# jspenmar/slowtv_monodepth

Measured on AMD Instinct MI355X. Metric: training images/sec (640×192, 3-frame) at 1/2/4/8 MI355X; warp+SSIM HBM GB/s, higher is better.
Workload: dtype f32

## Files before the change

### include/smd_hotpath.h

```cpp
#ifndef SMD_HOTPATH_H
#define SMD_HOTPATH_H

#include <stddef.h>
#include <stdint.h>

#ifdef __cplusplus
extern "C" {
#endif

#define SMD_ABI_VERSION 8

#define SMD_OK 0
#define SMD_E_INVALID (-1)
#define SMD_E_LAUNCH (-2)
#define SMD_E_WORKSPACE (-3)
#define SMD_E_UNSUPPORTED (-4)

#define SMD_USE_MIN 0x1
#define SMD_USE_AUTOMASK 0x2
#define SMD_LOSS_L1 0x4
#define SMD_NEED_K_GRAD 0x8
#define SMD_USE_EDGES 0x10
#define SMD_LOSS_L2 0x20
#define SMD_MASK_EXPLAINABILITY 0x80
#define SMD_MASK_UNCERTAINTY 0x100
#define SMD_BWD_SKIP_DEAD_ROWS 0x400
#define SMD_BWD_NO_LIVE 0x1000
#define SMD_USE_LAPLACIAN 0x200
#define SMD_EDGES_READY 0x800
#define SMD_PACKED_READY 0x40
#define SMD_REGR_L1 0x0
#define SMD_REGR_LOG_L1 0x1
#define SMD_REGR_BERHU 0x2
#define SMD_REGR_INVERT 0x4

#define SMD_MAX_SCALES 8
#define SMD_MAX_SUPPORTS 8
#define SMD_SEL_MASKED 255

const char* smd_last_error(void);
int smd_abi_version(void);

int smd_set_knob(const char* name, int value);
void smd_reset_knobs(void);

int smd_disp_to_depth_fwd(const float* const* disp, const int* hs, const int* ws, int S, int b, int h, int w,
                          float min_depth, float max_depth, float* depth_up, float* disp_up, void* stream);
size_t smd_disp_to_depth_workspace_bytes(const int* hs, const int* ws, int S, int b, int h, int w);
int smd_disp_to_depth_bwd(const int* hs, const int* ws, int S, int b, int h, int w, float min_depth, float max_depth,
                          const float* depth_up, const float* g_depth_up, float* const* g_disp,
                          void* workspace, size_t workspace_bytes, void* stream);

size_t smd_image_recon_workspace_bytes(int b, int n, int S, int h, int w);
size_t smd_packed_supports_bytes(int b, int n, int h, int w);
int smd_image_recon_prep(const float* tgt, const float* supp, float* supp_packed, const int* hs, const int* ws, int S,
                         int b, int n, int h, int w, int flags, void* stream);
int smd_image_recon_supports_per_pass(void);
int smd_image_recon_fwd(const float* depth, const float* tgt, const float* supp, const float* T, const float* K,
                        const float* K_inv, const float* noise, uint64_t seed, float* supp_packed, float* err, uint8_t* sel, float* loss,
                        float* warp0, void* workspace, size_t workspace_bytes,
                        int b, int n, int S, int h, int w, int flags, void* stream);
int smd_image_recon_bwd(const float* depth, const float* tgt, float* supp_packed, const float* T, const float* K,
                        const float* K_inv, const uint8_t* sel, const float* g_loss,
                        float* g_depth, float* g_T, float* g_K, float* g_Kinv, void* workspace, size_t workspace_bytes,
                        int b, int n, int S, int h, int w, int flags, void* stream);

size_t smd_image_recon_disp_workspace_bytes(const int* hs, const int* ws, int S, int b, int n, int h, int w);
int smd_image_recon_disp_fwd(const float* const* disp, const int* hs, const int* ws, int S, float min_depth, float max_depth,
                             const float* tgt, const float* supp, const float* T, const float* K, const float* K_inv,
                             const float* noise, uint64_t seed, float* supp_packed, float* depth_up, float* err, uint8_t* sel, float* loss,
                             float* warp0, void* workspace, size_t workspace_bytes, int b, int n, int h, int w, int flags, void* stream);
int smd_image_recon_disp_bwd(const int* hs, const int* ws, int S, float min_depth, float max_depth, const float* depth_up,
                             float* supp_packed, const float* T, const float* K, const float* K_inv, const uint8_t* sel,
                             const float* g_loss, const float* g_depth_up_in, float* const* g_disp, float* g_T, float* g_K, float* g_Kinv,
                             void* workspace, size_t workspace_bytes, int b, int n, int h, int w, int flags, void* stream);

size_t smd_loss_path_workspace_bytes(const int* hs, const int* ws, int S, int b, int n, int h, int w);
int smd_loss_path_fwd(const float* const* disp, const int* hs, const int* ws, const int* scale_keys, int S, float min_depth, float max_depth,
                      const float* tgt, const float* supp, const float* T, const float* K, const float* K_inv, uint64_t seed,
                      float* supp_packed, float* edge_weights, float* depth_up, uint8_t* sel, float* loss3, float* stats,
                      void* workspace, size_t workspace_bytes, int b, int n, int h, int w, int flags, float w_recon, float w_smooth, void* stream);
int smd_loss_path_bwd(const float* const* disp, const int* hs, const int* ws, const int* scale_keys, int S, float min_depth, float max_depth,
                      const float* depth_up, float* supp_packed, const float* T, const float* K, const float* K_inv, const uint8_t* sel,
                      const float* stats, const float* edge_weights, const float* g_loss, float w_recon, float w_smooth,
                      const float* aa, const float* t, const uint8_t* invert, const float* fs, const float* cs,
                      float* const* g_disp, float* g_T, float* g_K, float* g_Kinv, float* g_aa, float* g_t, float* g_fs, float* g_cs,
                      void* workspace, size_t workspace_bytes, int b, int n, int h, int w, int flags, void* stream);

int smd_gaussian_blur3x3(const float* x, float* out, int planes, int h, int w, int adjoint, void* stream);
size_t smd_disp_smooth_workspace_bytes(const int* hs, const int* ws, int S, int b);
size_t smd_disp_smooth_edge_weight_bytes(const int* hs, const int* ws, int S, int b);
int smd_disp_smooth_prep(const float* img, const int* hs, const int* ws, int S, int b, int h, int w, int flags, float* edge_weights, void* stream);
int smd_disp_smooth_fwd(const float* const* disp, const int* hs, const int* ws, const int* scale_keys, int S, int b,
                        const float* img, int h, int w, int flags, float* loss, float* stats, float* disp_grad, float* image_grad,
                        float* edge_weights, void* workspace, size_t workspace_bytes, void* stream);
int smd_disp_smooth_bwd(const float* const* disp, const int* hs, const int* ws, const int* scale_keys, int S, int b,
                        const float* img, int h, int w, int flags, const float* stats, const float* edge_weights,
                        const float* g_loss, float* const* g_disp, void* stream);

size_t smd_view_synth_workspace_bytes(int B, int h, int w);
int smd_view_synth_fwd(const float* input, const float* depth, const float* T, const float* K, const float* K_inv,
                       float* warp, float* depth_warp, uint8_t* mask_valid, int B, int C, int h, int w, void* stream);
int smd_view_synth_bwd(const float* input, const float* depth, const float* T, const float* K, const float* K_inv,
                       const float* g_warp, const float* g_depth_warp,
                       float* g_input, float* g_depth, float* g_T, float* g_K, float* g_Kinv,
                       void* workspace, size_t workspace_bytes, int B, int C, int h, int w, void* stream);

size_t smd_photo_error_workspace_bytes(int N, int C, int h, int w);
int smd_photo_error_fwd(const float* pred, const float* target, float* err, int N, int C, int h, int w, int flags, float weight_ssim, void* stream);
int smd_photo_error_bwd(const float* pred, const float* target, const float* g_err, float* g_pred,
                        void* workspace, size_t workspace_bytes, int N, int C, int h, int w, int flags, float weight_ssim, void* stream);

size_t smd_regression_workspace_bytes(size_t N);
int smd_regression_fwd(const float* pred, const float* target, const uint8_t* mask, size_t N, int flags, float* loss, float* err,
                       float* stats, void* workspace, size_t workspace_bytes, void* stream);
int smd_regression_bwd(const float* pred, const float* target, const uint8_t* mask, size_t N, int flags, float* stats,
                       const float* g_loss, float* g_pred, float* g_target, void* workspace, size_t workspace_bytes, void* stream);

size_t smd_recon_reduce_workspace_bytes(int B, int h, int w);
int smd_recon_reduce_fwd(const float* err_warp, const float* err_static, const float* mask, const float* noise, uint64_t seed,
                         float* err, uint8_t* sel, float* loss, void* workspace, size_t workspace_bytes,
                         int n, int B, int h, int w, int flags, void* stream);
int smd_recon_reduce_bwd(const uint8_t* sel, const float* g_loss, float* g_err_warp, const float* err_warp, const float* err_static,
                         const float* mask, float* g_mask, int n, int B, int h, int w, int flags, void* stream);

#define SMD_GLUE_A_BF16 1
#define SMD_GLUE_SKIP_BF16 2
#define SMD_GLUE_OUT_BF16 4
size_t smd_decoder_glue_workspace_bytes(int B, int C, int h, int w);
int smd_elu_pad_fwd(const void* x, const float* bias, void* out, int B, int C, int h, int w, int apply_elu, int dtypes, void* stream);
int smd_elu_pad_bwd(const void* x, const float* bias, const void* g_out, void* g_x, float* g_bias,
                    void* workspace, size_t workspace_bytes, int B, int C, int h, int w, int apply_elu, int dtypes, void* stream);
int smd_elu_up_cat_pad_fwd(const void* a, const float* bias, const void* skip, void* out, int B, int Ca, int Cs, int h, int w, int dtypes,
                           void* stream);
int smd_elu_up_cat_pad_bwd(const void* a, const float* bias, const void* g_out, void* g_a, void* g_skip, float* g_bias,
                           void* workspace, size_t workspace_bytes, int B, int Ca, int Cs, int h, int w, int dtypes, void* stream);

#define SMD_HEAD_X_BF16 2
size_t smd_conv3x3_head_workspace_bytes(int B, int C, int h, int w);
int smd_conv3x3_head_fwd(const void* xp, const float* weight, const float* bias, float* y, int B, int C, int h, int w, int act, void* stream);
int smd_conv3x3_head_bwd(const void* xp, const float* weight, const float* y, const float* g_y, void* g_xp, float* g_weight, float* g_bias,
                         void* workspace, size_t workspace_bytes, int B, int C, int h, int w, int act, void* stream);

#define SMD_HEADN_NONE 0
#define SMD_HEADN_SIGMOID 1
#define SMD_HEADN_RELU 2
#define SMD_HEADN_X_BF16 4
size_t smd_conv3x3_headn_workspace_bytes(int B, int C, int n, int h, int w);
int smd_conv3x3_headn_fwd(const void* xp, const float* weight, const float* bias, float* y, int B, int C, int n, int h, int w, int act, void* stream);
int smd_conv3x3_headn_bwd_data(const float* weight, const float* y, const float* g_y, void* g_xp, int B, int C, int n, int h, int w, int act, void* stream);
int smd_conv3x3_headn_bwd_wgt(const void* xp, const float* y, const float* g_y, float* g_weight, float* g_bias, void* workspace, size_t workspace_bytes,
                              int B, int C, int n, int h, int w, int act, void* stream);

int smd_upsample_stack_fwd(const float* const* x, const int* hs, const int* ws, int S, int b, int n, int h, int w, float* out, void* stream);
int smd_upsample_stack_bwd(const int* hs, const int* ws, int S, int b, int n, int h, int w, const float* g_out, float* const* g_x, void* stream);

#define SMD_MEAN_BCE_ONES 0
#define SMD_MEAN_IDENTITY 1
#define SMD_MEAN_NEGATE 2
size_t smd_scale_mean_workspace_bytes(const long long* numel, int S);
int smd_scale_mean_fwd(const float* const* x, const long long* numel, int S, int mode, float* loss, void* workspace, size_t workspace_bytes, void* stream);
int smd_scale_mean_bwd(const float* const* x, const long long* numel, int S, int mode, const float* g_loss, float* const* g_x, void* stream);

size_t smd_conv3x3_thin_workspace_bytes(int B, int C, int h, int w);
int smd_conv3x3_thin_fwd(const float* xp, const float* weight, float* y, int B, int C, int h, int w, void* stream);
int smd_conv3x3_thin_bwd(const float* xp, const float* weight, const float* g_y, float* g_xp, float* g_weight, void* workspace, size_t workspace_bytes,
                         int B, int C, int h, int w, void* stream);

size_t smd_conv3x3_mfma_packed_bytes(int C, int CO, int pieces);
size_t smd_conv3x3_mfma_workspace_bytes(int B, int C, int CO, int h, int w);
int smd_conv3x3_mfma_pack(const float* weight, void* wp_fwd, void* wp_bwd, int C, int CO, int pieces, void* stream);
int smd_conv3x3_mfma_fwd(const void* xp, const void* wp_fwd, void* y, void* workspace, size_t workspace_bytes,
                         int B, int C, int CO, int h, int w, int pieces, void* stream);
int smd_conv3x3_mfma_bwd_data(const void* g_y, const void* wp_bwd, void* g_xp, void* workspace, size_t workspace_bytes,
                              int B, int C, int CO, int h, int w, int pieces, void* stream);
int smd_conv3x3_mfma_bwd_weight(const void* xp, const void* g_y, float* g_weight, void* workspace, size_t workspace_bytes,
                                int B, int C, int CO, int h, int w, int pieces, void* stream);

size_t smd_conv3x3z_mfma_workspace_bytes(int B, int C, int CO, int h, int w);
int smd_conv3x3z_mfma_fwd(const float* x, const void* wp_fwd, float* y, void* workspace, size_t workspace_bytes,
                          int B, int C, int CO, int h, int w, int pieces, void* stream);
int smd_conv3x3z_mfma_bwd_data(const float* g_y, const void* wp_bwd, float* g_x, void* workspace, size_t workspace_bytes,
                               int B, int C, int CO, int h, int w, int pieces, void* stream);
int smd_conv3x3z_mfma_bwd_weight(const float* x, const float* g_y, float* g_weight, void* workspace, size_t workspace_bytes,
                                 int B, int C, int CO, int h, int w, int pieces, void* stream);

size_t smd_conv7x7s2_packed_bytes(int C, int CO);
size_t smd_conv7x7s2_workspace_bytes(int B, int C, int CO, int H, int W);
int smd_conv7x7s2_pack(const float* weight, void* wp, int C, int CO, void* stream);
int smd_conv7x7s2_fwd(const float* x, const void* wp, float* y, int B, int C, int CO, int H, int W, void* stream);
int smd_conv7x7s2_bwd_weight(const float* x, const float* g_y, float* g_weight, void* workspace, size_t workspace_bytes,
                             int B, int C, int CO, int H, int W, void* stream);

size_t smd_bn_workspace_bytes(int N, int C, int HW);
int smd_bn_fwd(const float* x, const float* residual, const float* gamma, const float* beta, float* running_mean, float* running_var,
               float momentum, float eps, int relu, float* y, float* save_mean, float* save_invstd,
               void* workspace, size_t workspace_bytes, int N, int C, int HW, void* stream);
int smd_bn_bwd(const float* x, const float* y, const float* g_y, const float* gamma, const float* save_mean, const float* save_invstd,
               int relu, float* g_x, float* g_residual, float* g_gamma, float* g_beta,
               void* workspace, size_t workspace_bytes, int N, int C, int HW, void* stream);

int smd_maxpool3x3s2_fwd(const float* x, float* y, uint8_t* idx, int N, int C, int H, int W, void* stream);
int smd_maxpool3x3s2_bwd(const float* g_y, const uint8_t* idx, float* g_x, int N, int C, int H, int W, void* stream);

size_t smd_dwconv7x7_workspace_bytes(int C, int H, int W);
int smd_dwconv7x7_fwd(const float* x, const float* weight, const float* bias, float* y, int N, int C, int H, int W, int flip, void* stream);
int smd_dwconv7x7_wrw(const float* x, const float* g_y, float* g_weight, float* g_bias, void* workspace, size_t workspace_bytes,
                      int N, int C, int H, int W, void* stream);

size_t smd_layernorm_cf_workspace_bytes(int N, int C, int HW);
int smd_layernorm_cf_fwd(const float* x, const float* gamma, const float* beta, void* y, int y_is_bf16, float* mean, float* rstd,
                         int N, int C, int HW, float eps, void* stream);
int smd_layernorm_cf_bwd(const float* x, const void* g_y, int g_y_is_bf16, const float* gamma, const float* mean, const float* rstd,
                         float* g_x, float* g_gamma, float* g_beta, void* workspace, size_t workspace_bytes, int N, int C, int HW, void* stream);

int smd_pose_fwd(const float* aa, const float* t, const uint8_t* invert, int N, float* T, void* stream);
int smd_pose_bwd(const float* aa, const float* t, const uint8_t* invert, int N, const float* g_T, float* g_aa, float* g_t, void* stream);
int smd_intrinsics_fwd(const float* fs, const float* cs, const float* K_in, int b, int h, int w, float* K, float* K_inv, void* stream);
int smd_intrinsics_bwd(const float* fs, const float* cs, int b, int h, int w, const float* g_K, const float* g_Kinv,
                       float* g_fs, float* g_cs, void* stream);

int smd_crop_resize(const float* const* src, float* const* dst, const int* planes, int nseg, int H, int W, int crop_h, int crop_w,
                    int out_h, int out_w, const float* K_in, float* K_out, int nK, void* stream);

#define SMD_PROF_RECON_FWD 0
#define SMD_PROF_RECON_BWD 1
#define SMD_PROF_RECON_FWD_ALL 2
#define SMD_PROF_RECON_BWD_ALL 3
#define SMD_PROF_RECON_PREP 4
const char* smd_last_kernel_variant(int which);
int smd_profile_enable(int which, int capacity);
int smd_profile_collect(int which, float* ms_out, int max_out, int* n_out);

int smd_debug_stream_copy(const void* src, void* dst, size_t nbytes, int mode, void* stream);

int smd_debug_lane_shift(float* out_left, float* out_right, void* stream);

#ifdef __cplusplus
}
#endif
#endif
```

### slowtv_monodepth_amd/_lib.py

```python
from __future__ import annotations

import ctypes as C
import os
from pathlib import Path

import torch

__all__ = ['lib', 'call', 'set_knob', 'reset_knobs', 'knob_epoch', 'lib_path', 'FLAGS', 'REGR_FLAGS', 'SEL_MASKED', 'ptr_array', 'int_array', 'i64_array', 'HotpathError', 'Unsupported']

_HERE = Path(__file__).resolve().parent
lib_path = Path(os.environ.get('SMD_HOTPATH_LIB', _HERE/'libsmd_hotpath.so'))

FLAGS = {'use_min': 0x1, 'use_automask': 0x2, 'loss_l1': 0x4, 'need_k_grad': 0x8, 'use_edges': 0x10, 'loss_l2': 0x20, 'packed_ready': 0x40,
         'mask_explainability': 0x80, 'mask_uncertainty': 0x100, 'use_laplacian': 0x200, 'bwd_skip_rows': 0x400, 'edges_ready': 0x800, 'bwd_no_live': 0x1000}
REGR_FLAGS = {'l1': 0x0, 'log_l1': 0x1, 'berhu': 0x2, 'invert': 0x4}
SEL_MASKED = 255
MAX_SCALES = 8
MAX_SUPPORTS = 8

_vp, _i, _f, _sz, _u64 = C.c_void_p, C.c_int, C.c_float, C.c_size_t, C.c_uint64

PROTOTYPES = {
    'smd_last_error': (C.c_char_p, []),
    'smd_abi_version': (_i, []),
    'smd_last_kernel_variant': (C.c_char_p, [_i]),
    'smd_set_knob': (_i, [C.c_char_p, _i]),
    'smd_reset_knobs': (None, []),
    'smd_disp_to_depth_fwd': (_i, [_vp, _vp, _vp, _i, _i, _i, _i, _f, _f, _vp, _vp, _vp]),
    'smd_disp_to_depth_workspace_bytes': (_sz, [_vp, _vp, _i, _i, _i, _i]),
    'smd_disp_to_depth_bwd': (_i, [_vp, _vp, _i, _i, _i, _i, _f, _f, _vp, _vp, _vp, _vp, _sz, _vp]),
    'smd_image_recon_workspace_bytes': (_sz, [_i, _i, _i, _i, _i]),
    'smd_packed_supports_bytes': (_sz, [_i, _i, _i, _i]),
    'smd_image_recon_prep': (_i, [_vp]*5 + [_i]*6 + [_vp]),
    'smd_image_recon_supports_per_pass': (_i, []),
    'smd_image_recon_fwd': (_i, [_vp]*7 + [_u64] + [_vp]*6 + [_sz] + [_i]*6 + [_vp]),
    'smd_image_recon_bwd': (_i, [_vp]*13 + [_sz] + [_i]*6 + [_vp]),
    'smd_image_recon_disp_workspace_bytes': (_sz, [_vp, _vp, _i, _i, _i, _i, _i]),
    'smd_image_recon_disp_fwd': (_i, [_vp, _vp, _vp, _i, _f, _f] + [_vp]*6 + [_u64] + [_vp]*7 + [_sz] + [_i]*5 + [_vp]),
    'smd_image_recon_disp_bwd': (_i, [_vp, _vp, _i, _f, _f] + [_vp]*13 + [_sz] + [_i]*5 + [_vp]),
    'smd_loss_path_workspace_bytes': (_sz, [_vp, _vp, _i, _i, _i, _i, _i]),
    'smd_loss_path_fwd': (_i, [_vp]*4 + [_i, _f, _f] + [_vp]*5 + [_u64] + [_vp]*7 + [_sz] + [_i]*5 + [_f, _f, _vp]),
    'smd_loss_path_bwd': (_i, [_vp]*4 + [_i, _f, _f] + [_vp]*9 + [_f, _f] + [_vp]*14 + [_sz] + [_i]*5 + [_vp]),
    'smd_disp_smooth_workspace_bytes': (_sz, [_vp, _vp, _i, _i]),
    'smd_disp_smooth_edge_weight_bytes': (_sz, [_vp, _vp, _i, _i]),
    'smd_gaussian_blur3x3': (_i, [_vp, _vp, _i, _i, _i, _i, _vp]),
    'smd_disp_smooth_prep': (_i, [_vp, _vp, _vp, _i, _i, _i, _i, _i, _vp, _vp]),
    'smd_disp_smooth_fwd': (_i, [_vp, _vp, _vp, _vp, _i, _i, _vp, _i, _i, _i, _vp, _vp, _vp, _vp, _vp, _vp, _sz, _vp]),
    'smd_disp_smooth_bwd': (_i, [_vp, _vp, _vp, _vp, _i, _i, _vp, _i, _i, _i, _vp, _vp, _vp, _vp, _vp]),
    'smd_view_synth_workspace_bytes': (_sz, [_i, _i, _i]),
    'smd_view_synth_fwd': (_i, [_vp]*8 + [_i]*4 + [_vp]),
    'smd_view_synth_bwd': (_i, [_vp]*13 + [_sz] + [_i]*4 + [_vp]),
    'smd_photo_error_workspace_bytes': (_sz, [_i, _i, _i, _i]),
    'smd_photo_error_fwd': (_i, [_vp]*3 + [_i]*5 + [_f, _vp]),
    'smd_photo_error_bwd': (_i, [_vp]*5 + [_sz] + [_i]*5 + [_f, _vp]),
    'smd_regression_workspace_bytes': (_sz, [_sz]),
    'smd_regression_fwd': (_i, [_vp]*3 + [_sz, _i] + [_vp]*4 + [_sz, _vp]),
    'smd_regression_bwd': (_i, [_vp]*3 + [_sz, _i] + [_vp]*5 + [_sz, _vp]),
    'smd_recon_reduce_workspace_bytes': (_sz, [_i, _i, _i]),
    'smd_recon_reduce_fwd': (_i, [_vp]*4 + [_u64] + [_vp]*4 + [_sz] + [_i]*5 + [_vp]),
    'smd_recon_reduce_bwd': (_i, [_vp]*7 + [_i]*5 + [_vp]),
    'smd_decoder_glue_workspace_bytes': (_sz, [_i]*4),
    'smd_conv3x3_headn_workspace_bytes': (_sz, [_i]*5),
    'smd_conv3x3_headn_fwd': (_i, [_vp]*4 + [_i]*6 + [_vp]),
    'smd_conv3x3_headn_bwd_data': (_i, [_vp]*4 + [_i]*6 + [_vp]),
    'smd_conv3x3_headn_bwd_wgt': (_i, [_vp]*6 + [_sz] + [_i]*6 + [_vp]),
    'smd_upsample_stack_fwd': (_i, [_vp]*3 + [_i]*5 + [_vp, _vp]),
    'smd_upsample_stack_bwd': (_i, [_vp]*2 + [_i]*5 + [_vp]*3),
    'smd_scale_mean_workspace_bytes': (_sz, [_vp, _i]),
    'smd_scale_mean_fwd': (_i, [_vp]*2 + [_i]*2 + [_vp]*2 + [_sz, _vp]),
    'smd_scale_mean_bwd': (_i, [_vp]*2 + [_i]*2 + [_vp]*3),
    'smd_conv3x3_thin_workspace_bytes': (_sz, [_i]*4),
    'smd_conv3x3_thin_fwd': (_i, [_vp]*3 + [_i]*4 + [_vp]),
    'smd_conv3x3_thin_bwd': (_i, [_vp]*6 + [_sz] + [_i]*4 + [_vp]),
    'smd_conv3x3_mfma_packed_bytes': (_sz, [_i]*3),
    'smd_conv3x3_mfma_workspace_bytes': (_sz, [_i]*5),
    'smd_conv3x3_mfma_pack': (_i, [_vp]*3 + [_i]*3 + [_vp]),
    'smd_conv3x3_mfma_fwd': (_i, [_vp]*4 + [_sz] + [_i]*6 + [_vp]),
    'smd_conv3x3_mfma_bwd_data': (_i, [_vp]*4 + [_sz] + [_i]*6 + [_vp]),
    'smd_conv3x3_mfma_bwd_weight': (_i, [_vp]*4 + [_sz] + [_i]*6 + [_vp]),
    'smd_conv3x3z_mfma_workspace_bytes': (_sz, [_i]*5),
    'smd_conv3x3z_mfma_fwd': (_i, [_vp]*4 + [_sz] + [_i]*6 + [_vp]),
    'smd_conv3x3z_mfma_bwd_data': (_i, [_vp]*4 + [_sz] + [_i]*6 + [_vp]),
    'smd_conv3x3z_mfma_bwd_weight': (_i, [_vp]*4 + [_sz] + [_i]*6 + [_vp]),
    'smd_conv7x7s2_packed_bytes': (_sz, [_i]*2),
    'smd_conv7x7s2_workspace_bytes': (_sz, [_i]*5),
    'smd_conv7x7s2_pack': (_i, [_vp]*2 + [_i]*2 + [_vp]),
    'smd_conv7x7s2_fwd': (_i, [_vp]*3 + [_i]*5 + [_vp]),
    'smd_conv7x7s2_bwd_weight': (_i, [_vp]*4 + [_sz] + [_i]*5 + [_vp]),
    'smd_conv3x3_head_workspace_bytes': (_sz, [_i]*4),
    'smd_conv3x3_head_fwd': (_i, [_vp]*4 + [_i]*5 + [_vp]),
    'smd_conv3x3_head_bwd': (_i, [_vp]*8 + [_sz] + [_i]*5 + [_vp]),
    'smd_elu_pad_fwd': (_i, [_vp]*3 + [_i]*6 + [_vp]),
    'smd_elu_pad_bwd': (_i, [_vp]*6 + [_sz] + [_i]*6 + [_vp]),
    'smd_elu_up_cat_pad_fwd': (_i, [_vp]*4 + [_i]*6 + [_vp]),
    'smd_elu_up_cat_pad_bwd': (_i, [_vp]*7 + [_sz] + [_i]*6 + [_vp]),
    'smd_bn_workspace_bytes': (_sz, [_i, _i, _i]),
    'smd_bn_fwd': (_i, [_vp]*6 + [_f, _f, _i] + [_vp]*4 + [_sz] + [_i]*3 + [_vp]),
    'smd_bn_bwd': (_i, [_vp]*6 + [_i] + [_vp]*5 + [_sz] + [_i]*3 + [_vp]),
    'smd_maxpool3x3s2_fwd': (_i, [_vp]*3 + [_i]*4 + [_vp]),
    'smd_maxpool3x3s2_bwd': (_i, [_vp]*3 + [_i]*4 + [_vp]),
    'smd_dwconv7x7_workspace_bytes': (_sz, [_i]*3),
    'smd_dwconv7x7_fwd': (_i, [_vp]*4 + [_i]*5 + [_vp]),
    'smd_dwconv7x7_wrw': (_i, [_vp]*5 + [_sz] + [_i]*4 + [_vp]),
    'smd_layernorm_cf_workspace_bytes': (_sz, [_i]*3),
    'smd_layernorm_cf_fwd': (_i, [_vp]*4 + [_i] + [_vp]*2 + [_i]*3 + [_f, _vp]),
    'smd_layernorm_cf_bwd': (_i, [_vp]*2 + [_i] + [_vp]*7 + [_sz] + [_i]*3 + [_vp]),
    'smd_pose_fwd': (_i, [_vp, _vp, _vp, _i, _vp, _vp]),
    'smd_pose_bwd': (_i, [_vp, _vp, _vp, _i, _vp, _vp, _vp, _vp]),
    'smd_intrinsics_fwd': (_i, [_vp, _vp, _vp, _i, _i, _i, _vp, _vp, _vp]),
    'smd_intrinsics_bwd': (_i, [_vp, _vp, _i, _i, _i, _vp, _vp, _vp, _vp, _vp]),
    'smd_crop_resize': (_i, [_vp, _vp, _vp] + [_i]*7 + [_vp, _vp, _i, _vp]),
    'smd_profile_enable': (_i, [_i, _i]),
    'smd_profile_collect': (_i, [_i, _vp, _i, _vp]),
    'smd_debug_stream_copy': (_i, [_vp, _vp, _sz, _i, _vp]),
    'smd_debug_lane_shift': (_i, [_vp, _vp, _vp]),
}


class HotpathError(RuntimeError):
    """A call into libsmd_hotpath.so returned a negative status."""


class Unsupported(HotpathError):
    """SMD_E_UNSUPPORTED: the entry point does not serve these arguments in this build (nothing was launched); the caller takes the general operators."""


def _load() -> C.CDLL:
    if not lib_path.is_file():
        raise ImportError(
            f'{lib_path} not found: the HIP hot path is not built. Run `python -c "import __graft_entry__ as g; g.build()"` '
            f'(or `make -C slowtv_monodepth_amd/csrc`). There is no CPU/PyTorch fallback for this path.')
    handle = C.CDLL(str(lib_path))
    for name, (res, args) in PROTOTYPES.items():
        fn = getattr(handle, name)
        fn.restype, fn.argtypes = res, args
    if handle.smd_abi_version() != 8: raise ImportError(f'ABI version mismatch in {lib_path}')
    return handle


lib = _load()


def call(name: str, *args):
    rc = getattr(lib, name)(*args)
    if rc != 0:
        msg = lib.smd_last_error().decode()
        if rc == -1: raise ValueError(f'{name}: {msg}')
        if rc == -4: raise Unsupported(f'{name}: {msg}')
        raise HotpathError(f'{name} failed ({rc}): {msg}')


def set_knob(name: str, value: int) -> bool:
    global knob_epoch
    rc = lib.smd_set_knob(name.encode(), int(value))
    if rc == -1: raise ValueError(lib.smd_last_error().decode())
    knob_epoch += 1
    return rc == 0


def reset_knobs() -> None:
    global knob_epoch
    lib.smd_reset_knobs()
    knob_epoch += 1


knob_epoch = 0


def ptr_array(ptrs):
    return (C.c_void_p*len(ptrs))(*ptrs)


def int_array(vals):
    return (C.c_int*len(vals))(*[int(v) for v in vals])


def i64_array(vals):
    return (C.c_longlong*len(vals))(*[int(v) for v in vals])
```

### slowtv_monodepth_amd/conv_ops.py

```python
from __future__ import annotations

from collections import namedtuple

import torch

from . import _lib
from ._device import _check, _check_fb, _on, _ptr, _stream, _workspace, call
from .conv_routing import serve

_BF = torch.bfloat16


def _thin_bwd(xp, weight, g_y, want_x, want_w):
    if not (want_x or want_w): return None, None
    B, C, H, W = xp.shape
    g_xp = torch.empty_like(xp) if want_x else None
    g_w = torch.empty_like(weight) if want_w else None
    ws, nbytes = _workspace(xp.device, _lib.lib.smd_conv3x3_thin_workspace_bytes, B, C, H - 2, W - 2, floor=256) if want_w else (None, 0)
    call('smd_conv3x3_thin_bwd', xp.data_ptr(), weight.data_ptr(), g_y.data_ptr(), _ptr(g_xp), _ptr(g_w), _ptr(ws), nbytes, B, C, H - 2, W - 2, _stream())
    return g_xp, g_w


class _Conv3x3Thin(torch.autograd.Function):
    @staticmethod
    def forward(ctx, xp, weight):
        xp = _check('xp', xp)
        if xp.ndim != 4 or xp.shape[2] < 4 or xp.shape[3] < 4: raise ValueError(f'expected a padded (B,C,h+2,w+2) with h, w >= 2, got {tuple(xp.shape)}')
        B, C, H, W = xp.shape
        weight = _check('weight', weight, (16, C, 3, 3))
        y = torch.empty((B, 16, H - 2, W - 2), device=xp.device, dtype=torch.float32)
        call('smd_conv3x3_thin_fwd', xp.data_ptr(), weight.data_ptr(), y.data_ptr(), B, C, H - 2, W - 2, _stream())
        ctx.save_for_backward(xp, weight)
        return y

    @staticmethod
    def backward(ctx, g_y):
        xp, weight = ctx.saved_tensors
        _on(xp)
        B, C, H, W = xp.shape
        g_y = _check('grad(y)', g_y, (B, 16, H - 2, W - 2))
        return _thin_bwd(xp, weight, g_y, *ctx.needs_input_grad)


def conv3x3_thin(xp, weight):
    return _Conv3x3Thin.apply(xp, weight)


_Served = namedtuple('_Served', 'fwd data wgt thin sized')


def _served(C, CO, zpad, sized) -> _Served:
    thin = CO == 16 and C in (16, 32) and not zpad
    return _Served(fwd=(C % 16 == 0 and CO % 32 == 0) or thin,
                   data=(CO % 16 == 0 and C % 32 == 0) or (C == 16 and CO == 16 and not zpad),
                   wgt=CO % 32 == 0 or thin, thin=thin, sized=sized)


def _mfma_pack(weight, C, CO, pieces, want_fwd, want_bwd):
    nbytes = _lib.lib.smd_conv3x3_mfma_packed_bytes(C, CO, pieces)
    wf = _workspace(weight.device, nbytes, floor=256)[0] if want_fwd else None
    wb = _workspace(weight.device, nbytes, floor=256)[0] if want_bwd else None
    call('smd_conv3x3_mfma_pack', weight.data_ptr(), _ptr(wf), _ptr(wb), C, CO, pieces, _stream())
    return wf, wb


def _mfma_ws_bytes(B, C, CO, h, w, zpad):
    return (_lib.lib.smd_conv3x3z_mfma_workspace_bytes if zpad else _lib.lib.smd_conv3x3_mfma_workspace_bytes)(B, C, CO, h, w)


def _mfma_launch(entry, zpad, a, b, out, nws, dims, pieces):
    ws, nws = _workspace(out.device, nws, floor=256)
    call(('smd_conv3x3z_mfma_' if zpad else 'smd_conv3x3_mfma_') + entry, a.data_ptr(), b.data_ptr(), out.data_ptr(), ws.data_ptr(), nws, *dims, pieces, _stream())
    return out


class _Conv3x3Wide(torch.autograd.Function):
    @staticmethod
    def forward(ctx, xp, weight, pieces, force, zpad=False):
        xp = _check_fb('xp', xp)
        if zpad and xp.dtype != torch.float32: raise TypeError(f'the zero-padded convolution takes float32 tensors, got {xp.dtype}')
        if xp.ndim != 4 or (not zpad and (xp.shape[2] < 3 or xp.shape[3] < 3)):
            raise ValueError(f'expected {"(B,C,h,w)" if zpad else "a padded (B,C,h+2,w+2)"}, got {tuple(xp.shape)}')
        B, C, H, W = xp.shape
        if weight.ndim != 4 or tuple(weight.shape[1:]) != (C, 3, 3): raise ValueError(f'weight: expected (CO,{C},3,3), got {tuple(weight.shape)}')
        CO = weight.shape[0]
        weight = _check('weight', weight, (CO, C, 3, 3))
        h, w = (H, W) if zpad else (H - 2, W - 2)
        dims = (B, C, CO, h, w)
        bf = xp.dtype == _BF
        if bf: pieces = 1
        nws = _mfma_ws_bytes(*dims, zpad)
        sv = _served(C, CO, zpad, force or nws > 0)
        if force and not sv.fwd:
            raise _lib.Unsupported(f'the MFMA forward serves C % 16 == 0 with CO % 32 == 0{"" if zpad else ", or CO = 16 with C = 16 | 32"}, not C={C} CO={CO}')
        y = torch.empty((B, CO, h, w), device=xp.device, dtype=xp.dtype)
        packed = {}

        def run_mfma():
            packed['wf'], packed['wb'] = _mfma_pack(weight, C, CO, pieces, True, sv.data)
            return _mfma_launch('fwd', zpad, xp, packed['wf'], y, nws, dims, pieces)

        def run_ref():
            if zpad: return torch.conv2d(xp, weight, None, 1, 1)
            if bf: return torch.conv2d(xp, weight.to(_BF))
            if sv.thin: call('smd_conv3x3_thin_fwd', xp.data_ptr(), weight.data_ptr(), y.data_ptr(), B, C, h, w, _stream()); return y
            return torch.conv2d(xp, weight)
        op = 'fwd_z' if zpad else 'fwd_bf16' if bf else 'fwd'
        out = serve((op, *dims), run_mfma, run_ref, eligible=sv.fwd and sv.sized, force=force)
        ctx.save_for_backward(xp, weight, packed.get('wb'))
        ctx.pieces, ctx.force, ctx.zpad, ctx.served = pieces, force, zpad, sv
        return out

    @staticmethod
    def backward(ctx, g_y):
        xp, weight, wp_bwd = ctx.saved_tensors
        _on(xp)
        B, C, H, W = xp.shape
        zpad, sv = ctx.zpad, ctx.served
        CO, pieces, force = weight.shape[0], ctx.pieces, ctx.force
        h, w = (H, W) if zpad else (H - 2, W - 2)
        dims = (B, C, CO, h, w)
        need_x, need_w = ctx.needs_input_grad[0], ctx.needs_input_grad[1]
        bf = xp.dtype == _BF
        g_y = _check_fb('grad(y)', g_y.to(xp.dtype), (B, CO, h, w))
        g_xp = g_w = None
        w_ref = weight.to(_BF) if bf else weight
        pad = [1, 1] if zpad else [0, 0]
        cb = lambda mask: torch.ops.aten.convolution_backward(g_y, xp, w_ref, None, [1, 1], pad, [1, 1], False, [0, 0], 1, mask)
        thin_ref = sv.thin and not bf
        sfx = '_z' if zpad else '_bf16' if bf else ''
        nws = _mfma_ws_bytes(*dims, zpad) if sv.sized and ((need_x and sv.data) or (need_w and sv.wgt)) else 0
        if need_x:
            g_xp = torch.empty_like(xp)
            packed = {'wb': wp_bwd}

            def run_data():
                if packed['wb'] is None: packed['wb'] = _mfma_pack(weight, C, CO, pieces, False, True)[1]
                return _mfma_launch('bwd_data', zpad, g_y, packed['wb'], g_xp, nws, dims, pieces)
            ref_data = (lambda: _thin_bwd(xp, weight, g_y, True, False)[0]) if thin_ref else (lambda: cb([True, False, False])[0])
            g_xp = serve(('data' + sfx, *dims), run_data, ref_data, eligible=sv.data and sv.sized, force=force)
        if need_w:
            g_w = torch.empty_like(weight)
            run_wgt = lambda: _mfma_launch('bwd_weight', zpad, xp, g_y, g_w, nws, dims, pieces)
            ref_wgt = (lambda: _thin_bwd(xp, weight, g_y, False, True)[1]) if thin_ref else (lambda: cb([False, True, False])[1].float())
            g_w = serve(('wgt' + sfx, *dims), run_wgt, ref_wgt, eligible=sv.wgt and sv.sized, force=force)
        return g_xp, g_w, None, None, None


def conv3x3_mfma(xp, weight, pieces: int = 3):
    return _Conv3x3Wide.apply(xp, weight, int(pieces), True)


def conv3x3_wide(xp, weight):
    return _Conv3x3Wide.apply(xp, weight, 3, False)


def conv3x3_same(x, weight):
    return _Conv3x3Wide.apply(x, weight, 3, False, True)


class _Conv7x7s2Stem(torch.autograd.Function):
    @staticmethod
    def forward(ctx, x, weight):
        x = _check('x', x)
        if x.ndim != 4: raise ValueError(f'expected (B,C,H,W), got {tuple(x.shape)}')
        B, C, H, W = x.shape
        if weight.ndim != 4 or tuple(weight.shape[1:]) != (C, 7, 7): raise ValueError(f'weight: expected (CO,{C},7,7), got {tuple(weight.shape)}')
        CO = weight.shape[0]
        weight = _check('weight', weight, (CO, C, 7, 7))
        ho, wo = (H - 1)//2 + 1, (W - 1)//2 + 1
        served = _lib.lib.smd_conv7x7s2_workspace_bytes(B, C, CO, H, W) > 0
        y = torch.empty((B, CO, ho, wo), device=x.device, dtype=torch.float32)

        def run_mfma():
            wp, _ = _workspace(x.device, _lib.lib.smd_conv7x7s2_packed_bytes, C, CO)
            call('smd_conv7x7s2_pack', weight.data_ptr(), wp.data_ptr(), C, CO, _stream())
            call('smd_conv7x7s2_fwd', x.data_ptr(), wp.data_ptr(), y.data_ptr(), B, C, CO, H, W, _stream())
            return y
        y = serve(('fwd_s', B, C, CO, H, W), run_mfma, lambda: torch.conv2d(x, weight, None, 2, 3), eligible=served)
        ctx.save_for_backward(x, weight)
        ctx.served = served
        return y

    @staticmethod
    def backward(ctx, g_y):
        x, weight = ctx.saved_tensors
        dev = _on(x)
        B, C, H, W = x.shape
        CO = weight.shape[0]
        need_x, need_w = ctx.needs_input_grad
        g_y = _check('grad(y)', g_y, (B, CO, (H - 1)//2 + 1, (W - 1)//2 + 1))
        cb = lambda mask: torch.ops.aten.convolution_backward(g_y, x, weight, None, [2, 2], [3, 3], [1, 1], False, [0, 0], 1, mask)
        g_x = cb([True, False, False])[0] if need_x else None
        g_w = None
        if need_w:
            g_w = torch.empty_like(weight)

            def run_wgt():
                ws, nws = _workspace(dev, _lib.lib.smd_conv7x7s2_workspace_bytes, B, C, CO, H, W, floor=256)
                call('smd_conv7x7s2_bwd_weight', x.data_ptr(), g_y.data_ptr(), g_w.data_ptr(), ws.data_ptr(), nws, B, C, CO, H, W, _stream())
                return g_w
            g_w = serve(('wgt_s', B, C, CO, H, W), run_wgt, lambda: cb([False, True, False])[1], eligible=ctx.served)
        return g_x, g_w


def conv7x7s2_stem(x, weight):
    return _Conv7x7s2Stem.apply(x, weight)
```

### slowtv_monodepth_amd/conv_routing.py

```python
from __future__ import annotations

import torch

from ._lib import Unsupported

_MODE = 'auto'
_ROUTES: dict = {}
_AB_WARMUPS, _AB_ROUNDS, _AB_MARGIN = 2, 5, 0.97
_DECLINED = (Unsupported, ValueError)


def set_conv_route(mode: str = 'auto'):
    global _MODE
    if mode not in ('auto', 'mfma', 'miopen'): raise ValueError(mode)
    _MODE = mode
    _ROUTES.clear()


def conv_routes() -> dict:
    return dict(_ROUTES)


_COARSE_W_MAX, _COARSE_C_MIN = 80, 256
_Z_FWD_WGT = [dict(px_min=1000, ch_max=511), dict(px_min=2400)]
STATIC_RULES = {
    'padded': {'fwd': [dict(thin=True), dict(thin=False, px_min=20000, c_co_max=128*64), dict(thin=False, coarse=True, px_min=1000)],
               'data': [dict(thin=True), dict(thin=False, px_min=5000, c_max=256), dict(thin=False, coarse=True, px_min=1000)],
               'wgt': [dict(thin=False, px_min=20000, co_max=64), dict(thin=False, coarse=True, px_min=2400)]},
    'bf16': {'fwd': [dict(thin=True)], 'data': [dict(thin=True)], 'wgt': [dict(thin=True)]},
    'zpad': {'fwd': _Z_FWD_WGT, 'data': [dict(px_min=1000)], 'wgt': _Z_FWD_WGT},
    'stem': {'fwd': [dict(px_min=20000)], 'wgt': [dict(px_min=20000)]},
}
_FAMILY_OF_SUFFIX = {'': 'padded', 'bf16': 'bf16', 'z': 'zpad', 's': 'stem'}
_BOUNDS = {'px_min': lambda v, B, C, CO, h, w: B*h*w >= v,
           'c_max': lambda v, B, C, CO, h, w: C <= v,
           'co_max': lambda v, B, C, CO, h, w: CO <= v,
           'c_co_max': lambda v, B, C, CO, h, w: C*CO <= v,
           'ch_max': lambda v, B, C, CO, h, w: max(C, CO) <= v,
           'thin': lambda v, B, C, CO, h, w: (CO == 16) == v,
           'coarse': lambda v, B, C, CO, h, w: (w <= _COARSE_W_MAX and C >= _COARSE_C_MIN) == v}


def static_rule(op, B, C, CO, h, w) -> bool:
    kind, _, suffix = op.partition('_')
    clauses = STATIC_RULES[_FAMILY_OF_SUFFIX[suffix]][kind]
    return any(all(_BOUNDS[name](v, B, C, CO, h, w) for name, v in clause.items()) for clause in clauses)


_capturing = torch.cuda.is_current_stream_capturing


def _time_interleaved(run_mfma, run_ref, rounds):
    ev = [[torch.cuda.Event(enable_timing=True) for _ in range(3)] for _ in range(rounds)]
    for e in ev:
        e[0].record(); run_mfma(); e[1].record(); run_ref(); e[2].record()
    torch.cuda.synchronize()
    return [e[0].elapsed_time(e[1])*1e3 for e in ev], [e[1].elapsed_time(e[2])*1e3 for e in ev]


def _conv_route(op, B, C, CO, h, w, run_mfma, run_ref) -> bool:
    if _MODE != 'auto': return _MODE == 'mfma'
    key = (op, B, C, CO, h, w)
    r = _ROUTES.get(key)
    if r is None:
        if _capturing(): return static_rule(op, B, C, CO, h, w)
        for _ in range(_AB_WARMUPS): run_mfma(); run_ref()
        us_m, us_r = _time_interleaved(run_mfma, run_ref, _AB_ROUNDS)
        t_m, t_r = sorted(us_m)[_AB_ROUNDS//2], sorted(us_r)[_AB_ROUNDS//2]
        r = _ROUTES[key] = (t_m < _AB_MARGIN*t_r, t_m, t_r)
    return r[0]


def serve(key, run_mfma, run_ref, *, eligible, force=False):
    if not eligible: return run_ref()
    if force: return run_mfma()
    try:
        use = _conv_route(*key, run_mfma, run_ref)
    except _DECLINED:
        _ROUTES[key] = (False, float('nan'), float('nan'))
        use = False
    if use:
        try:
            return run_mfma()
        except _DECLINED:
            pass
    return run_ref()
```

### slowtv_monodepth_amd/csrc/smd_api.hip

```cpp
#include <limits.h>
#include <stdarg.h>
#include <stdio.h>
#include <stdlib.h>
#include <string.h>
#include <algorithm>

#include "smd_kernels.h"
#include "smd_smooth_dev.h"

namespace {

thread_local char g_err[512] = "";

int fail(int code, const char* fmt, ...) {
  va_list ap;
  va_start(ap, fmt);
  vsnprintf(g_err, sizeof(g_err), fmt, ap);
  va_end(ap);
  return code;
}

int check_launch(hipError_t e, const char* what) {
  if (e != hipSuccess) return fail(SMD_E_LAUNCH, "%s: %s", what, hipGetErrorString(e));
  return SMD_OK;
// ... 620 lines not shown
int smd_photo_error_bwd(const float* pred, const float* target, const float* g_err, float* g_pred, void* workspace, size_t workspace_bytes,
                        int N, int C, int h, int w, int flags, float weight_ssim, void* stream) {
  if (!pred || !target || !g_err || !g_pred || !workspace) return fail(SMD_E_INVALID, "null pointer");
  if (N < 1 || N > 65535 || C < 1 || h < 2 || w < 2) return fail(SMD_E_INVALID, "invalid sizes N=%d C=%d h=%d w=%d", N, C, h, w);
  if (workspace_bytes < smd_photo_error_workspace_bytes(N, C, h, w)) return fail(SMD_E_WORKSPACE, "workspace too small");
  if (!(weight_ssim >= 0.f && weight_ssim <= 1.f)) return fail(SMD_E_INVALID, "Invalid SSIM weight. (%g vs. [0, 1])", weight_ssim);
  return check_launch(smd::launch_photo_error_bwd(pred, target, g_err, g_pred, (float*)workspace, N, C, h, w, flags, weight_ssim, (hipStream_t)stream), "photo_error_bwd");
}

size_t smd_regression_workspace_bytes(size_t N) {
  if (N < 1) return 0;
  return align256((size_t)smd::regr_blocks(N)*3*sizeof(float));
}

int smd_regression_fwd(const float* pred, const float* target, const uint8_t* mask, size_t N, int flags, float* loss, float* err, float* stats,
                       void* workspace, size_t workspace_bytes, void* stream) {
  if (!pred || !target || !loss || !stats || !workspace) return fail(SMD_E_INVALID, "null pointer");
  if (N < 1 || N > ((size_t)1 << 40)) return fail(SMD_E_INVALID, "invalid size N=%zu", N);
  if (workspace_bytes < smd_regression_workspace_bytes(N)) return fail(SMD_E_WORKSPACE, "workspace too small");
  return check_launch(smd::launch_regression_fwd(pred, target, mask, N, flags, loss, err, stats, (float*)workspace, (hipStream_t)stream), "regression_fwd");
}

int smd_regression_bwd(const float* pred, const float* target, const uint8_t* mask, size_t N, int flags, float* stats, const float* g_loss,
                       float* g_pred, float* g_target, void* workspace, size_t workspace_bytes, void* stream) {
  if (!pred || !target || !stats || !g_loss || !workspace || (!g_pred && !g_target)) return fail(SMD_E_INVALID, "null pointer");
  if (N < 1 || N > ((size_t)1 << 40)) return fail(SMD_E_INVALID, "invalid size N=%zu", N);
  if (workspace_bytes < smd_regression_workspace_bytes(N)) return fail(SMD_E_WORKSPACE, "workspace too small");
  return check_launch(smd::launch_regression_bwd(pred, target, mask, N, flags, stats, g_loss, g_pred, g_target, (float*)workspace, (hipStream_t)stream),
                      "regression_bwd");
}

size_t smd_recon_reduce_workspace_bytes(int B, int h, int w) {
  if (B < 1 || h < 1 || w < 1) return 0;
  return align256((size_t)smd::ceil_div(B*h*w, 256)*sizeof(float));
}

int smd_recon_reduce_fwd(const float* err_warp, const float* err_static, const float* mask, const float* noise, uint64_t seed, float* err, uint8_t* sel,
                         float* loss, void* workspace, size_t workspace_bytes, int n, int B, int h, int w, int flags, void* stream) {
  if (!err_warp || !err || !sel || !loss || !workspace) return fail(SMD_E_INVALID, "null pointer");
  if ((flags & (SMD_MASK_EXPLAINABILITY | SMD_MASK_UNCERTAINTY)) && !mask) return fail(SMD_E_INVALID, "Must provide a 'mask' when masking...");
  if ((flags & SMD_USE_AUTOMASK) && !err_static) return fail(SMD_E_INVALID, "Must provide the original 'source' images when automasking...");
  if (n < 1 || n >= SMD_SEL_MASKED || B < 1 || h < 1 || w < 1) return fail(SMD_E_INVALID, "invalid sizes");
  if (workspace_bytes < smd_recon_reduce_workspace_bytes(B, h, w)) return fail(SMD_E_WORKSPACE, "workspace too small");
  return check_launch(smd::launch_recon_reduce_fwd(err_warp, err_static, mask, noise, seed, err, sel, loss, (float*)workspace, n, B, h, w, flags,
                                                   (hipStream_t)stream), "recon_reduce_fwd");
}

int smd_recon_reduce_bwd(const uint8_t* sel, const float* g_loss, float* g_err_warp, const float* err_warp, const float* err_static,
                         const float* mask, float* g_mask, int n, int B, int h, int w, int flags, void* stream) {
  if (!sel || !g_loss || !g_err_warp) return fail(SMD_E_INVALID, "null pointer");
  if (n < 1 || B < 1 || h < 1 || w < 1) return fail(SMD_E_INVALID, "invalid sizes");
  if (mask && (!g_mask || !err_warp || ((flags & SMD_USE_AUTOMASK) && !err_static))) return fail(SMD_E_INVALID, "a masked reduction needs err_warp, err_static (with automask) and g_mask");
  return check_launch(smd::launch_recon_reduce_bwd(sel, g_loss, g_err_warp, err_warp, err_static, mask, g_mask, n, B, h, w, flags, (hipStream_t)stream), "recon_reduce_bwd");
}

static bool dec_sizes_ok(long long planes, int h, int w) {
  return planes >= 1 && h >= 2 && w >= 2 && (long long)(h + 2)*(w + 2) < (1ll << 30) && planes*(((long long)(h + 2)*(w + 2) + 255)/256) < (1ll << 31);
}
size_t smd_decoder_glue_workspace_bytes(int B, int C, int h, int w) {
  if (B < 1 || C < 1 || h < 1 || w < 1) return 0;
  return align256(smd::decoder_bias_partials(B, C, h, w)*sizeof(float));
}
int smd_elu_pad_fwd(const void* x, const float* bias, void* out, int B, int C, int h, int w, int apply_elu, int dtypes, void* stream) {
  if (!x || !out) return fail(SMD_E_INVALID, "null pointer");
  if (B < 1 || C < 1 || !dec_sizes_ok((long long)B*C, h, w)) return fail(SMD_E_INVALID, "invalid sizes B=%d C=%d h=%d w=%d", B, C, h, w);
  return check_launch(smd::launch_elu_pad_fwd(x, bias, out, B, C, h, w, apply_elu, dtypes, (hipStream_t)stream), "elu_pad_fwd");
}
int smd_elu_pad_bwd(const void* x, const float* bias, const void* g_out, void* g_x, float* g_bias, void* workspace, size_t workspace_bytes,
                    int B, int C, int h, int w, int apply_elu, int dtypes, void* stream) {
  if (!x || !g_out || !g_x || (g_bias && !workspace)) return fail(SMD_E_INVALID, "null pointer");
  if (B < 1 || C < 1 || !dec_sizes_ok((long long)B*C, h, w)) return fail(SMD_E_INVALID, "invalid sizes B=%d C=%d h=%d w=%d", B, C, h, w);
  if (g_bias && workspace_bytes < smd_decoder_glue_workspace_bytes(B, C, h, w)) return fail(SMD_E_WORKSPACE, "workspace too small");
  return check_launch(smd::launch_elu_pad_bwd(x, bias, g_out, g_x, g_bias, (float*)workspace, B, C, h, w, apply_elu, dtypes, (hipStream_t)stream), "elu_pad_bwd");
}
static bool head_sizes_ok(int B, int C, int h, int w) {
  return B >= 1 && C >= 1 && C < 65535 && dec_sizes_ok((long long)B*C, h, w) && (long long)B*((h + 47)/48) < 65536 && h < 65536 && (long long)B*C*(h + 2)*(w + 2) < (1ll << 40);
}
size_t smd_conv3x3_head_workspace_bytes(int B, int C, int h, int w) {
  if (!head_sizes_ok(B, C, h, w)) return 0;
  return align256(smd::conv_head_partials(B, C, h, w)*sizeof(float));
}
int smd_conv3x3_head_fwd(const void* xp, const float* weight, const float* bias, float* y, int B, int C, int h, int w, int act, void* stream) {
  if (!xp || !weight || !y) return fail(SMD_E_INVALID, "null pointer");
  if (!head_sizes_ok(B, C, h, w) || (act & ~(1 | SMD_HEAD_X_BF16))) return fail(SMD_E_INVALID, "invalid sizes B=%d C=%d h=%d w=%d act=%d", B, C, h, w, act);
  return check_launch(smd::launch_conv_head_fwd(xp, (act & SMD_HEAD_X_BF16) != 0, weight, bias, y, B, C, h, w, act & 1, (hipStream_t)stream), "conv3x3_head_fwd");
}
int smd_conv3x3_head_bwd(const void* xp, const float* weight, const float* y, const float* g_y, void* g_xp, float* g_weight, float* g_bias,
                         void* workspace, size_t workspace_bytes, int B, int C, int h, int w, int act, void* stream) {
  if (!weight || !y || !g_y || (!g_xp && !g_weight) || (g_weight && (!xp || !workspace)) || (g_bias && !g_weight)) return fail(SMD_E_INVALID, "null pointer");
  if (!head_sizes_ok(B, C, h, w) || (act & ~(1 | SMD_HEAD_X_BF16))) return fail(SMD_E_INVALID, "invalid sizes B=%d C=%d h=%d w=%d act=%d", B, C, h, w, act);
  if (g_weight && workspace_bytes < smd_conv3x3_head_workspace_bytes(B, C, h, w)) return fail(SMD_E_WORKSPACE, "workspace too small");
  return check_launch(smd::launch_conv_head_bwd(xp, (act & SMD_HEAD_X_BF16) != 0, weight, y, g_y, g_xp, g_weight, g_bias, (float*)workspace, B, C, h, w, act & 1, (hipStream_t)stream), "conv3x3_head_bwd");
}
static bool headn_args_ok(int B, int C, int n, int h, int w, int act) {
  const int a = act & 3;
  return n >= 1 && n <= 4 && head_sizes_ok(B, C, h, w) && (act & ~(3 | SMD_HEADN_X_BF16)) == 0 && a != 3 && dec_sizes_ok((long long)B*n, h, w);
}
size_t smd_conv3x3_headn_workspace_bytes(int B, int C, int n, int h, int w) {
  if (!headn_args_ok(B, C, n, h, w, 0)) return 0;
  return align256(smd::conv_headn_partials(B, C, n, h, w)*sizeof(float));
}
int smd_conv3x3_headn_fwd(const void* xp, const float* weight, const float* bias, float* y, int B, int C, int n, int h, int w, int act, void* stream) {
  if (!xp || !weight || !y) return fail(SMD_E_INVALID, "null pointer");
  if (!headn_args_ok(B, C, n, h, w, act)) return fail(SMD_E_INVALID, "invalid sizes B=%d C=%d n=%d h=%d w=%d act=%d (1 <= n <= 4)", B, C, n, h, w, act);
  return check_launch(smd::launch_conv_headn_fwd(xp, (act & SMD_HEADN_X_BF16) != 0, weight, bias, y, B, C, n, h, w, act & 3, (hipStream_t)stream), "conv3x3_headn_fwd");
}
int smd_conv3x3_headn_bwd_data(const float* weight, const float* y, const float* g_y, void* g_xp, int B, int C, int n, int h, int w, int act, void* stream) {
  if (!weight || !y || !g_y || !g_xp) return fail(SMD_E_INVALID, "null pointer");
  if (!headn_args_ok(B, C, n, h, w, act)) return fail(SMD_E_INVALID, "invalid sizes B=%d C=%d n=%d h=%d w=%d act=%d (1 <= n <= 4)", B, C, n, h, w, act);
  return check_launch(smd::launch_conv_headn_bwd(nullptr, (act & SMD_HEADN_X_BF16) != 0, weight, y, g_y, g_xp, nullptr, nullptr, nullptr, B, C, n, h, w, act & 3,
                                                 (hipStream_t)stream), "conv3x3_headn_bwd_data");
}
int smd_conv3x3_headn_bwd_wgt(const void* xp, const float* y, const float* g_y, float* g_weight, float* g_bias, void* workspace, size_t workspace_bytes,
                              int B, int C, int n, int h, int w, int act, void* stream) {
  if (!xp || !y || !g_y || !g_weight || !workspace) return fail(SMD_E_INVALID, "null pointer");
  if (!headn_args_ok(B, C, n, h, w, act)) return fail(SMD_E_INVALID, "invalid sizes B=%d C=%d n=%d h=%d w=%d act=%d (1 <= n <= 4)", B, C, n, h, w, act);
  if (workspace_bytes < smd_conv3x3_headn_workspace_bytes(B, C, n, h, w)) return fail(SMD_E_WORKSPACE, "workspace too small");
  return check_launch(smd::launch_conv_headn_bwd(xp, (act & SMD_HEADN_X_BF16) != 0, nullptr, y, g_y, nullptr, g_weight, g_bias, (float*)workspace, B, C, n, h, w, act & 3,
                                                 (hipStream_t)stream), "conv3x3_headn_bwd_wgt");
}

static int up_stack_check(int S, int b, int n, int h, int w) {
  if (b < 1 || n < 1 || h < 1 || w < 1 || (long long)b*n > 65535 || (long long)h*w >= (1ll << 30)) return fail(SMD_E_INVALID, "invalid sizes b=%d n=%d h=%d w=%d (b*n <= 65535)", b, n, h, w);
  if ((long long)S*b*n*h*w >= (1ll << 40)) return fail(SMD_E_INVALID, "output too large");
  return SMD_OK;
}
int smd_upsample_stack_fwd(const float* const* x, const int* hs, const int* ws, int S, int b, int n, int h, int w, float* out, void* stream) {
  if (!x || !out) return fail(SMD_E_INVALID, "null pointer");
  if (int rc = up_stack_check(S, b, n, h, w)) return rc;
  smd::ScaleSet sc;
  if (int rc = fill_scales(sc, x, nullptr, hs, ws, nullptr, S)) return rc;
  for (int s = 0; s < S; ++s) {
    if (!x[s]) return fail(SMD_E_INVALID, "null input pointer for scale %d", s);
    if ((long long)hs[s]*ws[s] >= (1ll << 30)) return fail(SMD_E_INVALID, "scale %d too large", s);
  }
  return check_launch(smd::launch_upsample_stack_fwd(sc, b*n, h, w, out, (hipStream_t)stream), "upsample_stack_fwd");
}
int smd_upsample_stack_bwd(const int* hs, const int* ws, int S, int b, int n, int h, int w, const float* g_out, float* const* g_x, void* stream) {
  if (!g_out || !g_x) return fail(SMD_E_INVALID, "null pointer");
  if (int rc = up_stack_check(S, b, n, h, w)) return rc;
  smd::ScaleSet sc;
  if (int rc = fill_scales(sc, nullptr, g_x, hs, ws, nullptr, S)) return rc;
  long long blocks = 0;
  for (int s = 0; s < S; ++s) {
    if (!g_x[s]) return fail(SMD_E_INVALID, "null gradient pointer for scale %d", s);
    if ((long long)hs[s]*ws[s] >= (1ll << 30)) return fail(SMD_E_INVALID, "scale %d too large", s);
    blocks += ((long long)hs[s]*ws[s] + 255)/256;
  }
  if (blocks >= (1ll << 31)) return fail(SMD_E_INVALID, "too many source pixels");
  return check_launch(smd::launch_upsample_stack_bwd(sc, b*n, h, w, g_out, (hipStream_t)stream), "upsample_stack_bwd");
}
static int fill_means(smd::MeanSet& ms, const float* const* x, float* const* g, const long long* numel, int S, int mode) {
  if (S < 1 || S > SMD_MAX_SCALES) return fail(SMD_E_INVALID, "S=%d outside [1, %d]", S, SMD_MAX_SCALES);
  if (!numel) return fail(SMD_E_INVALID, "null size array");
  if (mode < SMD_MEAN_BCE_ONES || mode > SMD_MEAN_NEGATE) return fail(SMD_E_INVALID, "invalid mode %d", mode);
  memset(&ms, 0, sizeof(ms));
  ms.S = S;
  for (int s = 0; s < S; ++s) {
    if (numel[s] < 1) return fail(SMD_E_INVALID, "scale %d is empty", s);
    ms.p[s] = x ? x[s] : nullptr; ms.g[s] = g ? g[s] : nullptr; ms.n[s] = numel[s];
  }
  if (smd::scale_mean_blocks(ms) < 1) return fail(SMD_E_INVALID, "too many elements");
  return SMD_OK;
}
size_t smd_scale_mean_workspace_bytes(const long long* numel, int S) {
  smd::MeanSet ms;
  if (fill_means(ms, nullptr, nullptr, numel, S, 0)) return 0;
  return 256 + align256((size_t)ms.first_block[SMD_MAX_SCALES]*sizeof(float));
}
int smd_scale_mean_fwd(const float* const* x, const long long* numel, int S, int mode, float* loss, void* workspace, size_t workspace_bytes, void* stream) {
  if (!x || !loss || !workspace) return fail(SMD_E_INVALID, "null pointer");
  smd::MeanSet ms;
  if (int rc = fill_means(ms, x, nullptr, numel, S, mode)) return rc;
  for (int s = 0; s < S; ++s) if (!x[s]) return fail(SMD_E_INVALID, "null input pointer for scale %d", s);
  if (workspace_bytes < smd_scale_mean_workspace_bytes(numel, S)) return fail(SMD_E_WORKSPACE, "workspace too small");
  return check_launch(smd::launch_scale_mean_fwd(ms, mode, (float*)((char*)workspace + 256), (unsigned*)workspace, loss, (hipStream_t)stream), "scale_mean_fwd");
}
int smd_scale_mean_bwd(const float* const* x, const long long* numel, int S, int mode, const float* g_loss, float* const* g_x, void* stream) {
  if (!g_loss || !g_x || (mode == SMD_MEAN_BCE_ONES && !x)) return fail(SMD_E_INVALID, "null pointer");
  smd::MeanSet ms;
  if (int rc = fill_means(ms, x, g_x, numel, S, mode)) return rc;
  for (int s = 0; s < S; ++s) if (!g_x[s] || (mode == SMD_MEAN_BCE_ONES && !x[s])) return fail(SMD_E_INVALID, "null pointer for scale %d", s);
  return check_launch(smd::launch_scale_mean_bwd(ms, mode, g_loss, (hipStream_t)stream), "scale_mean_bwd");
}
static bool thin_sizes_ok(int B, int C, int h, int w) { return (C == 16 || C == 32) && head_sizes_ok(B, C, h, w) && dec_sizes_ok((long long)B*16, h, w) && B < 65536 && h + 2 < 4*65536; }
size_t smd_conv3x3_thin_workspace_bytes(int B, int C, int h, int w) {
  if (!thin_sizes_ok(B, C, h, w)) return 0;
  return align256(smd::conv_thin_partials(B, C, h, w)*sizeof(float));
}
int smd_conv3x3_thin_bwd(const float* xp, const float* weight, const float* g_y, float* g_xp, float* g_weight, void* workspace, size_t workspace_bytes,
                         int B, int C, int h, int w, void* stream) {
  if (!g_y || (!g_xp && !g_weight) || (g_xp && !weight) || (g_weight && (!xp || !workspace))) return fail(SMD_E_INVALID, "null pointer");
  if (C != 16 && C != 32 && C >= 1) return fail(SMD_E_UNSUPPORTED, "the thin convolution serves 16 or 32 input channels, not %d", C);
  if (!thin_sizes_ok(B, C, h, w)) return fail(SMD_E_INVALID, "invalid sizes B=%d C=%d h=%d w=%d", B, C, h, w);
  if (g_weight && workspace_bytes < smd_conv3x3_thin_workspace_bytes(B, C, h, w)) return fail(SMD_E_WORKSPACE, "workspace too small");
  hipStream_t st = (hipStream_t)stream;
  if (g_xp) { if (int rc = check_launch(smd::launch_conv_thin_bwd_data(g_y, weight, g_xp, B, C, h, w, st), "conv3x3_thin_bwd (data)")) return rc; }
  if (g_weight) { if (int rc = check_launch(smd::launch_conv_thin_bwd_wgt(xp, g_y, g_weight, (float*)workspace, B, C, h, w, st), "conv3x3_thin_bwd (weights)")) return rc; }
  return SMD_OK;
}
int smd_conv3x3_thin_fwd(const float* xp, const float* weight, float* y, int B, int C, int h, int w, void* stream) {
  if (!xp || !weight || !y) return fail(SMD_E_INVALID, "null pointer");
  if (C != 16 && C != 32 && C >= 1) return fail(SMD_E_UNSUPPORTED, "the thin convolution serves 16 or 32 input channels, not %d", C);
  if (!thin_sizes_ok(B, C, h, w)) return fail(SMD_E_INVALID, "invalid sizes B=%d C=%d h=%d w=%d", B, C, h, w);
  return check_launch(smd::launch_conv_thin_fwd(xp, weight, y, B, C, h, w, (hipStream_t)stream), "conv3x3_thin_fwd");
}
static bool mfma_sizes_ok(int B, int C, int CO, int h, int w) {
  return B >= 1 && C >= 1 && CO >= 1 && C <= 4096 && CO <= 4096 && h >= 1 && w >= 1 && h < 32768 && w < 32768 && (long long)(h + 2)*(w + 2) < (1ll << 30) &&
         (long long)B*((C + 31)/32)*((CO + 31)/32) < 65536 && (long long)C*(h + 2)*(w + 2) < (1ll << 29) && (long long)CO*h*w < (1ll << 29);
}
using smd::ConvOp;
static bool conv_two_tiles() { return knob("conv_two_tiles", 0) != 0; }
size_t smd_conv3x3_mfma_packed_bytes(int C, int CO, int pieces) {
  if (C < 1 || CO < 1 || pieces < 1 || pieces > 3) return 0;
  return align256(smd::conv_mfma_packed_elems(C, CO, pieces)*2);
}
static size_t mfma_workspace_bytes(bool zpad, int B, int C, int CO, int h, int w, bool two_tiles) {
  if (!mfma_sizes_ok(B, C, CO, h, w)) return 0;
  size_t n = std::max({(size_t)64, smd::conv_mfma_split_elems(ConvOp::Fwd, zpad, B, C, CO, h, w, two_tiles), smd::conv_mfma_split_elems(ConvOp::Data, zpad, B, C, CO, h, w, two_tiles)});
  if (smd::conv_mfma_served(ConvOp::Wgt, zpad, C, CO)) n = std::max(n, smd::conv_mfma_wgrad_partials(zpad, B, C, CO, h, w));
  return align256(n*sizeof(float));
}
size_t smd_conv3x3_mfma_workspace_bytes(int B, int C, int CO, int h, int w) { return mfma_workspace_bytes(false, B, C, CO, h, w, conv_two_tiles()); }
size_t smd_conv3x3z_mfma_workspace_bytes(int B, int C, int CO, int h, int w) { return mfma_workspace_bytes(true, B, C, CO, h, w, conv_two_tiles()); }
static int mfma_unserved(ConvOp op, bool zpad, int C, int CO) {
  const char* name[] = {"forward", "data gradient", "weight gradient"};
  return fail(SMD_E_UNSUPPORTED, "the %s%s does not serve C=%d CO=%d", zpad ? "zero-padded " : "", name[(int)op], C, CO);
}
static int mfma_check(ConvOp op, bool zpad, size_t workspace_bytes, int B, int C, int CO, int h, int w, int pieces, bool two_tiles) {
  if (zpad && pieces != 2 && pieces != 3) return fail(SMD_E_UNSUPPORTED, "the zero-padded forms take float tensors: pieces 2 or 3, not %d", pieces);
  if (pieces < 1 || pieces > 3) return fail(SMD_E_UNSUPPORTED, "pieces must be 1 (bfloat16 tensors), 2 or 3 (float tensors), not %d", pieces);
  if (!mfma_sizes_ok(B, C, CO, h, w)) return fail(SMD_E_INVALID, "invalid sizes B=%d C=%d CO=%d h=%d w=%d", B, C, CO, h, w);
  if (!smd::conv_mfma_served(op, zpad, C, CO)) return mfma_unserved(op, zpad, C, CO);
  if (workspace_bytes < mfma_workspace_bytes(zpad, B, C, CO, h, w, two_tiles)) return fail(SMD_E_WORKSPACE, "workspace too small");
  return SMD_OK;
}
int smd_conv3x3_mfma_pack(const float* weight, void* wp_fwd, void* wp_bwd, int C, int CO, int pieces, void* stream) {
  if (!weight || (!wp_fwd && !wp_bwd)) return fail(SMD_E_INVALID, "null pointer");
  if (pieces < 1 || pieces > 3) return fail(SMD_E_UNSUPPORTED, "pieces must be 1 (bfloat16 tensors), 2 or 3 (float tensors), not %d", pieces);
  if (C < 1 || CO < 1 || C > 4096 || CO > 4096) return fail(SMD_E_INVALID, "invalid sizes C=%d CO=%d", C, CO);
  if (wp_fwd && !smd::conv_mfma_served(ConvOp::Fwd, false, C, CO)) return mfma_unserved(ConvOp::Fwd, false, C, CO);
  if (wp_bwd && !smd::conv_mfma_served(ConvOp::Data, false, C, CO)) return mfma_unserved(ConvOp::Data, false, C, CO);
  return check_launch(smd::launch_conv_mfma_pack(weight, wp_fwd, wp_bwd, C, CO, pieces, (hipStream_t)stream), "conv3x3_mfma_pack");
}
static int mfma_form(ConvOp op, bool zpad, const void* in, const void* wp, void* out, void* workspace, size_t workspace_bytes, int B, int C, int CO, int h, int w, int pieces, void* stream, const char* what) {
  if (!in || !wp || !out || !workspace) return fail(SMD_E_INVALID, "null pointer");
  const bool two_tiles = conv_two_tiles();
  if (int rc = mfma_check(op, zpad, workspace_bytes, B, C, CO, h, w, pieces, two_tiles)) return rc;
  const auto launch = op == ConvOp::Fwd ? smd::launch_conv_mfma_fwd : smd::launch_conv_mfma_bwd_data;
  return check_launch(launch(in, wp, out, (float*)workspace, zpad, B, C, CO, h, w, pieces, two_tiles, (hipStream_t)stream), what);
}
static int mfma_bwd_weight(bool zpad, const void* x, const void* g_y, float* g_weight, void* workspace, size_t workspace_bytes, int B, int C, int CO, int h, int w, int pieces, void* stream) {
  if (!x || !g_y || !g_weight || !workspace) return fail(SMD_E_INVALID, "null pointer");
  if (int rc = mfma_check(ConvOp::Wgt, zpad, workspace_bytes, B, C, CO, h, w, pieces, conv_two_tiles())) return rc;
  return check_launch(smd::launch_conv_mfma_bwd_wgt(x, g_y, g_weight, (float*)workspace, zpad, B, C, CO, h, w, pieces, (hipStream_t)stream), zpad ? "conv3x3z_mfma_bwd_weight" : "conv3x3_mfma_bwd_weight");
}
int smd_conv3x3_mfma_fwd(const void* xp, const void* wp_fwd, void* y, void* workspace, size_t workspace_bytes, int B, int C, int CO, int h, int w, int pieces, void* stream) {
  return mfma_form(ConvOp::Fwd, false, xp, wp_fwd, y, workspace, workspace_bytes, B, C, CO, h, w, pieces, stream, "conv3x3_mfma_fwd");
}
int smd_conv3x3_mfma_bwd_data(const void* g_y, const void* wp_bwd, void* g_xp, void* workspace, size_t workspace_bytes, int B, int C, int CO, int h, int w, int pieces, void* stream) {
  return mfma_form(ConvOp::Data, false, g_y, wp_bwd, g_xp, workspace, workspace_bytes, B, C, CO, h, w, pieces, stream, "conv3x3_mfma_bwd_data");
}
int smd_conv3x3_mfma_bwd_weight(const void* xp, const void* g_y, float* g_weight, void* workspace, size_t workspace_bytes, int B, int C, int CO, int h, int w, int pieces, void* stream) {
  return mfma_bwd_weight(false, xp, g_y, g_weight, workspace, workspace_bytes, B, C, CO, h, w, pieces, stream);
}
int smd_conv3x3z_mfma_fwd(const float* x, const void* wp_fwd, float* y, void* workspace, size_t workspace_bytes, int B, int C, int CO, int h, int w, int pieces, void* stream) {
  return mfma_form(ConvOp::Fwd, true, x, wp_fwd, y, workspace, workspace_bytes, B, C, CO, h, w, pieces, stream, "conv3x3z_mfma_fwd");
}
int smd_conv3x3z_mfma_bwd_data(const float* g_y, const void* wp_bwd, float* g_x, void* workspace, size_t workspace_bytes, int B, int C, int CO, int h, int w, int pieces, void* stream) {
  return mfma_form(ConvOp::Data, true, g_y, wp_bwd, g_x, workspace, workspace_bytes, B, C, CO, h, w, pieces, stream, "conv3x3z_mfma_bwd_data");
}
int smd_conv3x3z_mfma_bwd_weight(const float* x, const float* g_y, float* g_weight, void* workspace, size_t workspace_bytes, int B, int C, int CO, int h, int w, int pieces, void* stream) {
  return mfma_bwd_weight(true, x, g_y, g_weight, workspace, workspace_bytes, B, C, CO, h, w, pieces, stream);
}
static bool stem_sizes_ok(int B, int C, int H, int W) {
  if (B < 1 || B > 65535 || C < 1 || H < 1 || W < 1) return false;
  const long long ho = (H - 1)/2 + 1, wo = (W - 1)/2 + 1;
  return (long long)C*H*W < (1ll << 31) && 64*ho*wo < (1ll << 31) && (ho + 3)/4 <= 65535;
}
size_t smd_conv7x7s2_packed_bytes(int C, int CO) { return smd::conv_stem_served(C, CO) ? smd::conv_stem_packed_bytes(C) : 0; }
size_t smd_conv7x7s2_workspace_bytes(int B, int C, int CO, int H, int W) {
  if (!smd::conv_stem_served(C, CO) || !stem_sizes_ok(B, C, H, W)) return 0;
  return align256(smd::conv_stem_wgrad_floats(B, C, H, W)*sizeof(float));
}
int smd_conv7x7s2_pack(const float* weight, void* wp, int C, int CO, void* stream) {
  if (!weight || !wp) return fail(SMD_E_INVALID, "null pointer");
  if (!smd::conv_stem_served(C, CO)) return fail(SMD_E_UNSUPPORTED, "the stem kernels serve CO == 64 with C == 3 | 6, not C=%d CO=%d", C, CO);
  return check_launch(smd::launch_conv_stem_pack(weight, wp, C, (hipStream_t)stream), "conv7x7s2_pack");
}
int smd_conv7x7s2_fwd(const float* x, const void* wp, float* y, int B, int C, int CO, int H, int W, void* stream) {
  if (!x || !wp || !y) return fail(SMD_E_INVALID, "null pointer");
  if (!smd::conv_stem_served(C, CO)) return fail(SMD_E_UNSUPPORTED, "the stem kernels serve CO == 64 with C == 3 | 6, not C=%d CO=%d", C, CO);
  if (!stem_sizes_ok(B, C, H, W)) return fail(SMD_E_INVALID, "invalid sizes B=%d C=%d H=%d W=%d", B, C, H, W);
  return check_launch(smd::launch_conv_stem_fwd(x, wp, y, B, C, H, W, (hipStream_t)stream), "conv7x7s2_fwd");
}
int smd_conv7x7s2_bwd_weight(const float* x, const float* g_y, float* g_weight, void* workspace, size_t workspace_bytes,
                             int B, int C, int CO, int H, int W, void* stream) {
  if (!x || !g_y || !g_weight || !workspace) return fail(SMD_E_INVALID, "null pointer");
  if (!smd::conv_stem_served(C, CO)) return fail(SMD_E_UNSUPPORTED, "the stem kernels serve CO == 64 with C == 3 | 6, not C=%d CO=%d", C, CO);
  if (!stem_sizes_ok(B, C, H, W)) return fail(SMD_E_INVALID, "invalid sizes B=%d C=%d H=%d W=%d", B, C, H, W);
  if (workspace_bytes < smd_conv7x7s2_workspace_bytes(B, C, CO, H, W)) return fail(SMD_E_WORKSPACE, "workspace too small");
  return check_launch(smd::launch_conv_stem_bwd_wgt(x, g_y, g_weight, (float*)workspace, B, C, H, W, (hipStream_t)stream), "conv7x7s2_bwd_weight");
}
int smd_elu_up_cat_pad_fwd(const void* a, const float* bias, const void* skip, void* out, int B, int Ca, int Cs, int h, int w, int dtypes, void* stream) {
  if (!a || !out || (Cs > 0 && !skip)) return fail(SMD_E_INVALID, "null pointer");
  if (B < 1 || Ca < 1 || Cs < 0 || h < 1 || w < 1 || !dec_sizes_ok((long long)B*(Ca + Cs), 2*h, 2*w))
    return fail(SMD_E_INVALID, "invalid sizes B=%d Ca=%d Cs=%d h=%d w=%d", B, Ca, Cs, h, w);
  return check_launch(smd::launch_elu_up_cat_pad_fwd(a, bias, skip, out, B, Ca, Cs, h, w, dtypes, (hipStream_t)stream), "elu_up_cat_pad_fwd");
}
int smd_elu_up_cat_pad_bwd(const void* a, const float* bias, const void* g_out, void* g_a, void* g_skip, float* g_bias,
                           void* workspace, size_t workspace_bytes, int B, int Ca, int Cs, int h, int w, int dtypes, void* stream) {
  if (!a || !g_out || (!g_a && !g_skip) || (g_bias && (!workspace || !g_a))) return fail(SMD_E_INVALID, "null pointer");
  if (B < 1 || Ca < 1 || Cs < 0 || h < 1 || w < 1 || !dec_sizes_ok((long long)B*(Ca + Cs), 2*h, 2*w))
    return fail(SMD_E_INVALID, "invalid sizes B=%d Ca=%d Cs=%d h=%d w=%d", B, Ca, Cs, h, w);
  if (g_bias && workspace_bytes < smd_decoder_glue_workspace_bytes(B, Ca, h, w)) return fail(SMD_E_WORKSPACE, "workspace too small");
  return check_launch(smd::launch_elu_up_cat_pad_bwd(a, bias, g_out, g_a, g_skip, g_bias, (float*)workspace, B, Ca, Cs, h, w, dtypes, (hipStream_t)stream),
                      "elu_up_cat_pad_bwd");
}

size_t smd_bn_workspace_bytes(int N, int C, int HW) {
  if (N < 1 || C < 1 || HW < 1) return 0;
  return align256(((size_t)C*smd::bn_chunks(N, HW)*2 + (size_t)C*3)*sizeof(float));
}
int smd_bn_fwd(const float* x, const float* residual, const float* gamma, const float* beta, float* running_mean, float* running_var,
               float momentum, float eps, int relu, float* y, float* save_mean, float* save_invstd, void* workspace, size_t workspace_bytes,
               int N, int C, int HW, void* stream) {
  if (!x || !gamma || !beta || !y || !save_mean || !save_invstd || !workspace) return fail(SMD_E_INVALID, "null pointer");
  if (N < 1 || C < 1 || C > 65535 || HW < 1 || (long long)N*HW < 2) return fail(SMD_E_INVALID, "invalid sizes N=%d C=%d HW=%d", N, C, HW);
  if (workspace_bytes < smd_bn_workspace_bytes(N, C, HW)) return fail(SMD_E_WORKSPACE, "workspace too small");
  return check_launch(smd::launch_bn_fwd(x, residual, gamma, beta, running_mean, running_var, momentum, eps, relu, y, save_mean, save_invstd,
                                         (float*)workspace, N, C, HW, (hipStream_t)stream), "bn_fwd");
}
int smd_bn_bwd(const float* x, const float* y, const float* g_y, const float* gamma, const float* save_mean, const float* save_invstd, int relu,
               float* g_x, float* g_residual, float* g_gamma, float* g_beta, void* workspace, size_t workspace_bytes, int N, int C, int HW,
               void* stream) {
  if (!x || !g_y || !gamma || !save_mean || !save_invstd || !g_x || !g_gamma || !g_beta || !workspace || (relu && !y))
    return fail(SMD_E_INVALID, "null pointer");
  if (N < 1 || C < 1 || C > 65535 || HW < 1) return fail(SMD_E_INVALID, "invalid sizes N=%d C=%d HW=%d", N, C, HW);
  if (workspace_bytes < smd_bn_workspace_bytes(N, C, HW)) return fail(SMD_E_WORKSPACE, "workspace too small");
  return check_launch(smd::launch_bn_bwd(x, y, g_y, gamma, save_mean, save_invstd, relu, g_x, g_residual, g_gamma, g_beta, (float*)workspace,
                                         N, C, HW, (hipStream_t)stream), "bn_bwd");
}

int smd_maxpool3x3s2_fwd(const float* x, float* y, uint8_t* idx, int N, int C, int H, int W, void* stream) {
  if (!x || !y || !idx) return fail(SMD_E_INVALID, "null pointer");
  if (N < 1 || C < 1 || H < 1 || W < 1 || (long long)N*C*(((long long)H*W + 1023)/1024) >= (1ll << 31)) return fail(SMD_E_INVALID, "invalid sizes");
  return check_launch(smd::launch_maxpool_fwd(x, y, idx, (size_t)N*C, H, W, (hipStream_t)stream), "maxpool_fwd");
}
int smd_maxpool3x3s2_bwd(const float* g_y, const uint8_t* idx, float* g_x, int N, int C, int H, int W, void* stream) {
  if (!g_y || !idx || !g_x) return fail(SMD_E_INVALID, "null pointer");
  if (N < 1 || C < 1 || H < 1 || W < 1 || (long long)N*C*(((long long)H*W + 1023)/1024) >= (1ll << 31)) return fail(SMD_E_INVALID, "invalid sizes");
  return check_launch(smd::launch_maxpool_bwd(g_y, idx, g_x, (size_t)N*C, H, W, (hipStream_t)stream), "maxpool_bwd");
}

static bool dw_sizes_ok(int N, int C, int H, int W) {
  return N >= 1 && C >= 1 && H >= 1 && W >= 1 && (long long)N*C*smd::dwconv_tiles(H, W) < (1ll << 31) && (long long)H*W < (1ll << 30);
}
size_t smd_dwconv7x7_workspace_bytes(int C, int H, int W) {
  if (C < 1 || H < 1 || W < 1) return 0;
  return align256((size_t)C*smd::dwconv_tiles(H, W)*50*sizeof(float));
}
int smd_dwconv7x7_fwd(const float* x, const float* weight, const float* bias, float* y, int N, int C, int H, int W, int flip, void* stream) {
  if (!x || !weight || !y) return fail(SMD_E_INVALID, "null pointer");
  if (!dw_sizes_ok(N, C, H, W)) return fail(SMD_E_INVALID, "invalid sizes N=%d C=%d H=%d W=%d", N, C, H, W);
  return check_launch(smd::launch_dwconv7(x, weight, bias, y, N, C, H, W, flip, (hipStream_t)stream), "dwconv7x7_fwd");
}
int smd_dwconv7x7_wrw(const float* x, const float* g_y, float* g_weight, float* g_bias, void* workspace, size_t workspace_bytes,
                      int N, int C, int H, int W, void* stream) {
  if (!x || !g_y || !g_weight || !workspace) return fail(SMD_E_INVALID, "null pointer");
  if (!dw_sizes_ok(N, C, H, W)) return fail(SMD_E_INVALID, "invalid sizes N=%d C=%d H=%d W=%d", N, C, H, W);
  if (workspace_bytes < smd_dwconv7x7_workspace_bytes(C, H, W)) return fail(SMD_E_WORKSPACE, "workspace too small");
  return check_launch(smd::launch_dwconv7_wrw(x, g_y, g_weight, g_bias, (float*)workspace, N, C, H, W, (hipStream_t)stream), "dwconv7x7_wrw");
}

size_t smd_layernorm_cf_workspace_bytes(int N, int C, int HW) {
  if (N < 1 || C < 1 || HW < 1) return 0;
  return align256((size_t)smd::ln_cf_chunks((size_t)N*HW)*C*2*sizeof(float));
}
int smd_layernorm_cf_fwd(const float* x, const float* gamma, const float* beta, void* y, int y_is_bf16, float* mean, float* rstd, int N, int C, int HW,
                         float eps, void* stream) {
  if (!x || !gamma || !beta || !y || !mean || !rstd) return fail(SMD_E_INVALID, "null pointer");
  if (N < 1 || C < 1 || HW < 1 || (long long)N*HW >= (1ll << 38)) return fail(SMD_E_INVALID, "invalid sizes N=%d C=%d HW=%d", N, C, HW);
  return check_launch(smd::launch_ln_cf_fwd(x, gamma, beta, y, y_is_bf16, mean, rstd, N, C, HW, eps, (hipStream_t)stream), "layernorm_cf_fwd");
}
int smd_layernorm_cf_bwd(const float* x, const void* g_y, int g_y_is_bf16, const float* gamma, const float* mean, const float* rstd, float* g_x, float* g_gamma,
                         float* g_beta, void* workspace, size_t workspace_bytes, int N, int C, int HW, void* stream) {
  if (!x || !g_y || !gamma || !mean || !rstd || !g_x || !g_gamma || !g_beta || !workspace) return fail(SMD_E_INVALID, "null pointer");
  if (N < 1 || C < 1 || C > 32767 || HW < 1) return fail(SMD_E_INVALID, "invalid sizes N=%d C=%d HW=%d", N, C, HW);
  if (workspace_bytes < smd_layernorm_cf_workspace_bytes(N, C, HW)) return fail(SMD_E_WORKSPACE, "workspace too small");
  return check_launch(smd::launch_ln_cf_bwd(x, g_y, g_y_is_bf16, gamma, mean, rstd, g_x, g_gamma, g_beta, (float*)workspace, N, C, HW, (hipStream_t)stream),
                      "layernorm_cf_bwd");
}

int smd_pose_fwd(const float* aa, const float* t, const uint8_t* invert, int N, float* T, void* stream) {
  if (!aa || !t || !T) return fail(SMD_E_INVALID, "null pointer");
  if (N < 1) return fail(SMD_E_INVALID, "invalid size N=%d", N);
  return check_launch(smd::launch_pose_fwd(aa, t, invert, N, T, (hipStream_t)stream), "pose_fwd");
}
int smd_pose_bwd(const float* aa, const float* t, const uint8_t* invert, int N, const float* g_T, float* g_aa, float* g_t, void* stream) {
  if (!aa || !t || !g_T || !g_aa || !g_t) return fail(SMD_E_INVALID, "null pointer");
  if (N < 1) return fail(SMD_E_INVALID, "invalid size N=%d", N);
  return check_launch(smd::launch_pose_bwd(aa, t, invert, N, g_T, g_aa, g_t, (hipStream_t)stream), "pose_bwd");
}
int smd_intrinsics_fwd(const float* fs, const float* cs, const float* K_in, int b, int h, int w, float* K, float* K_inv, void* stream) {
  if (!K_inv || (fs && (!cs || !K)) || (!fs && !K_in)) return fail(SMD_E_INVALID, "null pointer");
  if (b < 1 || h < 1 || w < 1) return fail(SMD_E_INVALID, "invalid sizes");
  return check_launch(smd::launch_intrinsics_fwd(fs, cs, K_in, b, h, w, K, K_inv, (hipStream_t)stream), "intrinsics_fwd");
}
int smd_intrinsics_bwd(const float* fs, const float* cs, int b, int h, int w, const float* g_K, const float* g_Kinv,
                       float* g_fs, float* g_cs, void* stream) {
  if (!fs || !cs || !g_K || !g_Kinv || !g_fs || !g_cs) return fail(SMD_E_INVALID, "null pointer");
  if (b < 1 || h < 1 || w < 1) return fail(SMD_E_INVALID, "invalid sizes");
  return check_launch(smd::launch_intrinsics_bwd(fs, cs, b, h, w, g_K, g_Kinv, g_fs, g_cs, (hipStream_t)stream), "intrinsics_bwd");
}

int smd_crop_resize(const float* const* src, float* const* dst, const int* planes, int nseg, int H, int W, int crop_h, int crop_w,
                    int out_h, int out_w, const float* K_in, float* K_out, int nK, void* stream) {
  if (!src || !dst || !planes) return fail(SMD_E_INVALID, "null pointer");
  if (nseg < 1 || nseg > smd::SMD_MAX_AR_SEGMENTS) return fail(SMD_E_INVALID, "nseg=%d outside [1, %d]", nseg, smd::SMD_MAX_AR_SEGMENTS);
  if (H < 2 || W < 2 || crop_h < 1 || crop_w < 1 || crop_h > H || crop_w > W || out_h < 1 || out_w < 1)
    return fail(SMD_E_INVALID, "invalid sizes: input %dx%d, crop %dx%d, output %dx%d", H, W, crop_h, crop_w, out_h, out_w);
  if ((K_in != nullptr) != (K_out != nullptr) || (K_in && nK < 1)) return fail(SMD_E_INVALID, "K_in / K_out / nK must be given together");
  smd::CropResizeArgs a;
  memset(&a, 0, sizeof(a));
  long long total = 0;
  for (int k = 0; k < nseg; ++k) {
    if (!src[k] || !dst[k] || planes[k] < 1) return fail(SMD_E_INVALID, "segment %d: null pointer or no planes", k);
    a.src[k] = src[k]; a.dst[k] = dst[k]; a.planes[k] = planes[k]; a.first_plane[k] = (int)total;
    total += planes[k];
  }
  if (total + 1 > 65535) return fail(SMD_E_INVALID, "too many image planes for one launch (%lld)", total);
  a.nseg = nseg; a.H = H; a.W = W; a.ch = crop_h; a.cw = crop_w; a.oh = out_h; a.ow = out_w;
  a.y0 = (int)((double)H/2.0 - (double)crop_h/2.0); a.x0 = (int)((double)W/2.0 - (double)crop_w/2.0);
  a.resample = (crop_h != H || crop_w != W) ? 1 : 0;
  a.K_in = K_in; a.K_out = K_out; a.nK = nK;
  return check_launch(smd::launch_crop_resize(a, (hipStream_t)stream), "crop_resize");
}

int smd_profile_enable(int which, int capacity) {
  if (which < 0 || which > 4 || capacity < 0) return fail(SMD_E_INVALID, "bad profile slot");
  ProfSlot& p = g_prof[which];
  for (int i = 0; i < 2*p.cap; ++i) (void)hipEventDestroy(p.ev[i]);
  delete[] p.ev;
  p = ProfSlot();
  if (capacity == 0) return SMD_OK;
  p.ev = new hipEvent_t[2*capacity];
  for (int i = 0; i < 2*capacity; ++i)
    if (hipEventCreate(&p.ev[i]) != hipSuccess) return fail(SMD_E_LAUNCH, "hipEventCreate failed");
  p.cap = capacity;
  return SMD_OK;
}

int smd_profile_collect(int which, float* ms_out, int max_out, int* n_out) {
  if (which < 0 || which > 4 || !ms_out || !n_out) return fail(SMD_E_INVALID, "bad profile arguments");
  ProfSlot& p = g_prof[which];
  int n = 0;
  for (int i = 0; i < p.used && n < max_out; ++i) {
    if (hipEventSynchronize(p.ev[2*i + 1]) != hipSuccess) return fail(SMD_E_LAUNCH, "hipEventSynchronize failed");
    float ms = 0.f;
    if (hipEventElapsedTime(&ms, p.ev[2*i], p.ev[2*i + 1]) != hipSuccess) return fail(SMD_E_LAUNCH, "hipEventElapsedTime failed");
    ms_out[n++] = ms;
  }
  p.used = 0;
  *n_out = n;
  return SMD_OK;
}

int smd_debug_stream_copy(const void* src, void* dst, size_t nbytes, int mode, void* stream) {
  if (!src || !dst) return fail(SMD_E_INVALID, "null pointer");
  if (nbytes < 16 || (nbytes & 15) || ((uintptr_t)src & 15) || ((uintptr_t)dst & 15)) return fail(SMD_E_INVALID, "size and pointers must be multiples of 16");
  return check_launch(smd::launch_stream_copy(src, dst, nbytes, mode, (hipStream_t)stream), "stream_copy");
}

int smd_debug_lane_shift(float* out_left, float* out_right, void* stream) {
  if (!out_left || !out_right) return fail(SMD_E_INVALID, "null pointer");
  return check_launch(smd::launch_debug_lane_shift(out_left, out_right, (hipStream_t)stream), "debug_lane_shift");
}

}
```

### slowtv_monodepth_amd/csrc/smd_conv_mfma.hip

```cpp
#include "smd_common.h"
#include "smd_kernels.h"
#include "smd_split_dev.h"
#include <algorithm>
#include <type_traits>

namespace smd {

template <int P> __device__ __forceinline__ void split_pair(unsigned short a, unsigned short b, unsigned (&p)[P]) {
  static_assert(P == 1, "bfloat16 operands have one piece");
  p[0] = (unsigned)a | ((unsigned)b << 16);
}
template <typename T> struct RawOf { typedef float type; };
template <> struct RawOf<bf16> { typedef unsigned short type; };
template <typename T> __device__ __forceinline__ void store_out(T* p, size_t i, float v);
template <> __device__ __forceinline__ void store_out<float>(float* p, size_t i, float v) { p[i] = v; }
template <> __device__ __forceinline__ void store_out<bf16>(bf16* p, size_t i, float v) { p[i] = __float2bfloat16(v); }

template <int P>
__global__ __launch_bounds__(256) void k_conv_pack_w(const float* __restrict__ w, unsigned short* __restrict__ wp_fwd, unsigned short* __restrict__ wp_bwd, int CO, int C) {
  const int idx = blockIdx.x*256 + threadIdx.x;
  if (idx >= CO*C*9) return;
  const int tap = idx % 9, c = (idx/9) % C, co = idx/(9*C);
  unsigned pk[P];
  split_pair<P>(w[idx], 0.f, pk);
// ... 812 lines not shown
  bf16x8 A[3][P];
#pragma unroll
  for (int r = 0; r < 3; ++r)
#pragma unroll
    for (int p = 0; p < P; ++p) A[r][p] = as_frag(uint4{0u, 0u, 0u, 0u});

  auto step = [&](int i, bf16x8 (&a0)[P], const bf16x8 (&a1)[P], const bf16x8 (&a2)[P]) {
    const int after = min(D - 2, nsteps - 1 - i);
    if (after >= 2) asm volatile("s_waitcnt vmcnt(%0)" :: "n"(2*NDMA) : "memory");
    else if (after == 1) asm volatile("s_waitcnt vmcnt(%0)" :: "n"(NDMA) : "memory");
    else asm volatile("s_waitcnt vmcnt(0)" ::: "memory");
    __builtin_amdgcn_s_barrier();
    asm volatile("" ::: "memory");
    if (i + D - 1 < nsteps) issue(i + D - 1);
    const float* slot = reinterpret_cast<const float*>(lds) + (i % D)*SLOT;
    const float* xr = slot + (nc*16 + j)*CS + ks*32 + q*8;
    const float* gr = slot + XDW + j*CS + ks*32 + q*8;
    const float4 x0v = *reinterpret_cast<const float4*>(xr), x1v = *reinterpret_cast<const float4*>(xr + 4);
    const float2 x2v = *reinterpret_cast<const float2*>(xr + 8);
    const float4 g0v = *reinterpret_cast<const float4*>(gr), g1v = *reinterpret_cast<const float4*>(gr + 4);
    unsigned px[5][P], pg[4][P];
    split_pair<P>(x0v.x, x0v.y, px[0]); split_pair<P>(x0v.z, x0v.w, px[1]); split_pair<P>(x1v.x, x1v.y, px[2]); split_pair<P>(x1v.z, x1v.w, px[3]); split_pair<P>(x2v.x, x2v.y, px[4]);
    split_pair<P>(g0v.x, g0v.y, pg[0]); split_pair<P>(g0v.z, g0v.w, pg[1]); split_pair<P>(g1v.x, g1v.y, pg[2]); split_pair<P>(g1v.z, g1v.w, pg[3]);
    bf16x8 Bx[3][P];
#pragma unroll
    for (int p = 0; p < P; ++p) {
      Bx[0][p] = as_frag(uint4{px[0][p], px[1][p], px[2][p], px[3][p]});
      Bx[1][p] = as_frag(uint4{__builtin_amdgcn_alignbit(px[1][p], px[0][p], 16), __builtin_amdgcn_alignbit(px[2][p], px[1][p], 16),
                               __builtin_amdgcn_alignbit(px[3][p], px[2][p], 16), __builtin_amdgcn_alignbit(px[4][p], px[3][p], 16)});
      Bx[2][p] = as_frag(uint4{px[1][p], px[2][p], px[3][p], px[4][p]});
      a0[p] = as_frag(i < nrows ? uint4{pg[0][p], pg[1][p], pg[2][p], pg[3][p]} : uint4{0u, 0u, 0u, 0u});
    }
#pragma unroll
    for (int ky = 0; ky < 3; ++ky) {
      const bf16x8 (&a)[P] = ky == 0 ? a0 : ky == 1 ? a1 : a2;
#pragma unroll
      for (int t = 0; t < NPROD; ++t)
#pragma unroll
        for (int kx = 0; kx < 3; ++kx) acc[ky*3 + kx] = __builtin_amdgcn_mfma_f32_16x16x32_bf16(a[prod_a(P, t)], Bx[kx][prod_b(P, t)], acc[ky*3 + kx], 0, 0, 0);
    }
  };

  static_assert(D == 4, "the waits above");
#pragma unroll
  for (int r = 0; r < D - 1; ++r) issue(r);
  for (int i = 0; i < nsteps; i += 3) {
    step(i, A[0], A[2], A[1]);
    if (i + 1 < nsteps) step(i + 1, A[1], A[0], A[2]);
    if (i + 2 < nsteps) step(i + 2, A[2], A[1], A[0]);
  }
  __syncthreads();
  float* red = reinterpret_cast<float*>(lds);
  if (ks == 1) {
#pragma unroll
    for (int t = 0; t < 9; ++t)
#pragma unroll
      for (int v = 0; v < 4; ++v) red[(nc*36 + t*4 + v)*64 + lane] = acc[t][v];
  }
  __syncthreads();
  if (ks == 0) {
    const size_t blk = ((size_t)b*gridDim.y + blockIdx.y)*gridDim.x + blockIdx.x;
#pragma unroll
    for (int t = 0; t < 9; ++t)
#pragma unroll
      for (int v = 0; v < 4; ++v) {
        const int co = 4*q + v, c = nc*16 + j;
        partial[((blk*9 + t)*16 + co)*C + c] = acc[t][v] + red[(nc*36 + t*4 + v)*64 + lane];
      }
  }
}

template <bool DIRECT>
__global__ __launch_bounds__(256) void k_conv_wgrad_finalize(const float* __restrict__ partial, unsigned T, unsigned G, int CO, int C, double* __restrict__ slice, float* __restrict__ g_w) {
  __shared__ double part[4][64];
  const int lane = threadIdx.x & 63, wv = threadIdx.x >> 6;
  const int n = CO*C*9, i = blockIdx.x*64 + lane;
  const unsigned g = blockIdx.y, t0 = (unsigned)(((unsigned long long)T*g)/G), t1 = (unsigned)(((unsigned long long)T*(g + 1))/G);
  double s = 0.0;
  if (i < n) for (unsigned t = t0 + wv; t < t1; t += 4) s += (double)partial[(size_t)t*n + i];
  part[wv][lane] = s;
  __syncthreads();
  if (wv == 0 && i < n) {
    const double tot = (part[0][lane] + part[1][lane]) + (part[2][lane] + part[3][lane]);
    if (DIRECT) { const int c = i % C, co = (i/C) % CO, tap = i/(C*CO); g_w[((size_t)co*C + c)*9 + tap] = (float)tot; }
    else slice[(size_t)g*n + i] = tot;
  }
}
__global__ __launch_bounds__(256) void k_conv_wgrad_finalize2(const double* __restrict__ slice, unsigned G, int CO, int C, float* __restrict__ g_w) {
  const int n = CO*C*9, i = blockIdx.x*256 + threadIdx.x;
  if (i >= n) return;
  double tot = 0.0;
  unsigned g = 0;
  for (; g + 8 <= G; g += 8) {
    double v[8];
#pragma unroll
    for (int k = 0; k < 8; ++k) v[k] = slice[(size_t)(g + k)*n + i];
#pragma unroll
    for (int k = 0; k < 8; ++k) tot += v[k];
  }
  for (; g < G; ++g) tot += slice[(size_t)g*n + i];
  const int c = i % C, co = (i/C) % CO, tap = i/(C*CO);
  g_w[((size_t)co*C + c)*9 + tap] = (float)tot;
}
static unsigned wgrad_slices(unsigned T) { return T < 64 ? 1u : std::min(32u, T/16); }

static void wgrad_shape(int B, int C, int CO, int h, int w, dim3& grid, int& rows, int& spb, bool multi) {
  const int cgs = ceil_div(C, 64)*(CO/32), strips = ceil_div(w, 32), base = strips*B*cgs;
  const int groups = std::max(1, std::min(512/std::max(base, 1), ceil_div(h, 12)));
  rows = ceil_div(h, groups);
  spb = 1;
  if (multi && rows == h && base > 512) {
    const long long per = (long long)strips*cgs;
    long long best = -1;
    for (int s = 1; s <= B; ++s) {
      const long long nsg = ceil_div(B, s), cost = ceil_div(nsg*per, 256ll)*(s*(h + 2) + 4);
      if (s > 1 && nsg*per < 512) break;
      if (best < 0 || cost < best) { best = cost; spb = s; }
    }
  }
  grid = dim3(strips, ceil_div(h, rows), ceil_div(B, spb)*cgs);
}
static void wgrad_shape(int B, int C, int CO, int h, int w, dim3& grid, int& rows) { int spb; wgrad_shape(B, C, CO, h, w, grid, rows, spb, false); }
static void wgrad16_shape(int B, int C, int h, int w, dim3& grid, int& rows) {
  const int strips = ceil_div(w, 64);
  const long long units = (long long)strips*B, slots = C == 16 ? 1024 : 768;
  const int groups = (int)std::max(1ll, std::min<long long>(ceil_div(h, 12), slots/units));
  rows = ceil_div(h, groups);
  grid = dim3(strips, ceil_div(h, rows), B);
}
static unsigned wgrad_sets(int B, int C, int CO, int h, int w, bool multi) {
  dim3 grid; int rows, spb = 1;
  if (CO == 16) wgrad16_shape(B, C, h, w, grid, rows); else wgrad_shape(B, C, CO, h, w, grid, rows, spb, multi);
  return grid.x*grid.y*(unsigned)ceil_div(B, spb);
}
static size_t wgrad_floats(unsigned T, int C, int CO) {
  const size_t n = (size_t)9*CO*C;
  const unsigned G = wgrad_slices(T);
  return (size_t)T*n + (G > 1 ? 2*(size_t)G*n : 0);
}
size_t conv_mfma_wgrad_partials(bool zpad, int B, int C, int CO, int h, int w) { return wgrad_floats(wgrad_sets(B, C, CO, h, w, zpad), C, CO); }
static size_t thin_packed_elems(int C, int pieces) { return (size_t)(C >> 4)*5*pieces*512; }
size_t conv_mfma_packed_elems(int C, int CO, int pieces) { return std::max((size_t)CO*C*9*pieces, CO == 16 ? thin_packed_elems(C, pieces) : (size_t)0); }

#define SMD_BY_PIECES(pieces, CALL) do { if ((pieces) == 3) { CALL(3, float); } else if ((pieces) == 2) { CALL(2, float); } else { CALL(1, bf16); } } while (0)

template <int P, typename T>
static void launch_conv16(const void* in, const void* wp, void* out, int B, int CK, bool bwd, int hi, int wi, int ho, int wo, hipStream_t st) {
  const unsigned gx = ceil_div(wo, 64), gy = ceil_div(ho, 4), gz = B;
  const dim3 grid(8*(unsigned)ceil_div((long long)gx*gy*gz, 8ll));
  const uint4* wq = (const uint4*)wp;
  const T* i_ = (const T*)in; T* o_ = (T*)out;
  if (bwd) hipLaunchKernelGGL((k_conv16_mfma<1, P, true, T, T>), grid, dim3(256), 0, st, i_, wq, o_, hi, wi, ho, wo, gx, gy, gz);
  else if (CK == 16) hipLaunchKernelGGL((k_conv16_mfma<1, P, false, T, T>), grid, dim3(256), 0, st, i_, wq, o_, hi, wi, ho, wo, gx, gy, gz);
  else hipLaunchKernelGGL((k_conv16_mfma<2, P, false, T, T>), grid, dim3(256), 0, st, i_, wq, o_, hi, wi, ho, wo, gx, gy, gz);
}

hipError_t launch_conv_mfma_pack(const float* w, void* wp_fwd, void* wp_bwd, int C, int CO, int pieces, hipStream_t st) {
  if (CO == 16) {
    void* thin_bwd = (C == 16) ? wp_bwd : nullptr;
    if (wp_fwd || thin_bwd) {
      const dim3 g16(ceil_div((C >> 4)*5*512, 256));
#define SMD_CALL(P, T) hipLaunchKernelGGL((k_conv_pack_w16<P>), g16, dim3(256), 0, st, w, (unsigned short*)wp_fwd, (unsigned short*)thin_bwd, C)
      SMD_BY_PIECES(pieces, SMD_CALL);
#undef SMD_CALL
    }
    if (C == 16 || !wp_bwd) return hipGetLastError();
    wp_fwd = nullptr;
  }
  const dim3 grid(ceil_div(CO*C*9, 256));
#define SMD_CALL(P, T) hipLaunchKernelGGL((k_conv_pack_w<P>), grid, dim3(256), 0, st, w, (unsigned short*)wp_fwd, (unsigned short*)wp_bwd, CO, C)
  SMD_BY_PIECES(pieces, SMD_CALL);
#undef SMD_CALL
  return hipGetLastError();
}

struct ConvShape { int TC, TRB, NM, KS, kcs, S; unsigned gx, gy, gz; dim3 grid; size_t out_elems; };
static double band_shape(int B, int CK, int ho, int wo, int& BR, int& S) {
  constexpr int NP = ConvTile<0>::NPIX;
  const int PW = wo + 2;
  if (3*PW > NP || (long long)B*CK*(ho + 2)*PW >= (1ll << 31)) return 0.0;
  if (ho*wo <= 128) {
    BR = ho; S = std::min(256/(ho*wo), B);
    while (S > 1 && S*(ho + 2)*PW > NP) --S;
  } else {
    S = 1; BR = std::min(ho, 256/wo);
    while (BR > 0 && (BR + 2)*PW > NP) --BR;
    if (BR == 0) return 0.0;
  }
  return (double)B*ho*wo/((double)ceil_div(ho, BR)*ceil_div(B, S)*256.0);
}
static ConvShape conv_shape(int B, int CK, int M, int ho, int wo, bool two_tiles) {
  ConvShape s;
  s.TC = wo >= 48 ? 64 : 32; s.TRB = wo >= 48 ? 4 : 8; s.S = 1;
  const int KC = CK >> 4;
  {
    const double rect = (double)B*ho*wo/((double)ceil_div(wo, s.TC)*s.TC*ceil_div(ho, s.TRB)*s.TRB*B);
    int BR = 0, S = 1;
    const double band = rect < 0.9 ? band_shape(B, CK, ho, wo, BR, S) : 0.0;
    if (band > rect + 0.05) {
      s.TC = 0; s.TRB = BR; s.S = S; s.NM = 1;
      s.gx = BR; s.gy = ceil_div(ho, BR); s.gz = ceil_div(B, S);
      s.out_elems = (size_t)B*M*ho*wo;
      const long long base = (long long)s.gy*s.gz*(M/32);
      double best = -1.0;
      for (int kcs = std::min(2, KC); kcs <= KC; ++kcs) {
        const int KS = ceil_div(KC, kcs);
        if (ceil_div(KC, KS) != kcs) continue;
        const double cost = (double)ceil_div(base*KS, 512ll)*(kcs + 1) + (KS > 1 ? (2.0*KS + 1.0)*s.out_elems*4.0/25e6 : 0.0);
        if (best < 0.0 || cost < best - 1e-9) { best = cost; s.kcs = kcs; s.KS = KS; }
      }
      s.grid = dim3(8*(unsigned)ceil_div(base*s.KS, 8ll));
      return s;
    }
  }
  const long long tiles = (long long)ceil_div(wo, s.TC)*ceil_div(ho, s.TRB)*B;
  s.NM = (M % 64 == 0 && tiles*(M/64) >= 256 && two_tiles) ? 2 : 1;
  const long long base = tiles*(M/(32*s.NM));
  int ks = 1;
  if (base < 384) ks = (int)std::min<long long>(std::max(KC/2, 1), (512 + base - 1)/base);
  s.kcs = ceil_div(KC, ks); s.KS = ceil_div(KC, s.kcs);
  s.gx = ceil_div(wo, s.TC); s.gy = ceil_div(ho, s.TRB); s.gz = B;
  s.grid = dim3(8*(unsigned)ceil_div((long long)s.gx*s.gy*s.gz*(M/(32*s.NM))*s.KS, 8ll));
  s.out_elems = (size_t)B*M*ho*wo;
  return s;
}
size_t conv_mfma_split_elems(ConvOp op, bool zpad, int B, int C, int CO, int h, int w, bool two_tiles) {
  if (op == ConvOp::Wgt || !conv_mfma_served(op, zpad, C, CO) || (CO == 16 && (op == ConvOp::Fwd || C == 16))) return 0;
  const int e = zpad ? 0 : 2;
  const ConvShape s = op == ConvOp::Fwd ? conv_shape(B, C, CO, h, w, two_tiles) : conv_shape(B, CO, C, h + e, w + e, two_tiles);
  return s.KS > 1 ? (size_t)s.KS*s.out_elems : 0;
}

template <int P, int OFF, typename T>
static void launch_conv_form(const void* in, const void* wp, void* out, float* split_ws, int B, int CK, int M, int hi, int wi, int ho, int wo, bool two_tiles, hipStream_t st) {
  const ConvShape s = conv_shape(B, CK, M, ho, wo, two_tiles);
  const uint4* wq = (const uint4*)wp;
  const T* i_ = (const T*)in;
  T* dst = s.KS > 1 ? reinterpret_cast<T*>(split_ws) : (T*)out;
  if (s.TC == 0) hipLaunchKernelGGL((k_conv_mfma<0, P, OFF, T, T, 1>), s.grid, dim3(256), 0, st, i_, wq, dst, CK, M, hi, wi, ho, wo, s.KS, s.kcs, s.out_elems, s.gx, s.gy, s.gz, s.S, B);
  else if (s.NM == 2) {
    if (s.TC == 64) hipLaunchKernelGGL((k_conv_mfma<64, P, OFF, T, T, 2>), s.grid, dim3(512), 0, st, i_, wq, dst, CK, M, hi, wi, ho, wo, s.KS, s.kcs, s.out_elems, s.gx, s.gy, s.gz, 1, B);
    else hipLaunchKernelGGL((k_conv_mfma<32, P, OFF, T, T, 2>), s.grid, dim3(512), 0, st, i_, wq, dst, CK, M, hi, wi, ho, wo, s.KS, s.kcs, s.out_elems, s.gx, s.gy, s.gz, 1, B);
  } else if (s.TC == 64) hipLaunchKernelGGL((k_conv_mfma<64, P, OFF, T, T, 1>), s.grid, dim3(256), 0, st, i_, wq, dst, CK, M, hi, wi, ho, wo, s.KS, s.kcs, s.out_elems, s.gx, s.gy, s.gz, 1, B);
  else hipLaunchKernelGGL((k_conv_mfma<32, P, OFF, T, T, 1>), s.grid, dim3(256), 0, st, i_, wq, dst, CK, M, hi, wi, ho, wo, s.KS, s.kcs, s.out_elems, s.gx, s.gy, s.gz, 1, B);
  if (s.KS > 1) {
    const size_t n4 = s.out_elems/4;
    hipLaunchKernelGGL((k_conv_split_sum<T>), dim3((unsigned)((n4 + 255)/256)), dim3(256), 0, st, split_ws, (T*)out, n4, s.KS);
  }
}

#define SMD_BY_PIECES_F32(pieces, CALL) do { if ((pieces) == 3) { CALL(3); } else { CALL(2); } } while (0)
hipError_t launch_conv_mfma_fwd(const void* x, const void* wp_fwd, void* y, float* split_ws, bool zpad, int B, int C, int CO, int h, int w, int pieces, bool two_tiles, hipStream_t st) {
  if (zpad) {
#define SMD_CALL(P) launch_conv_form<P, 1, float>(x, wp_fwd, y, split_ws, B, C, CO, h, w, h, w, two_tiles, st)
    SMD_BY_PIECES_F32(pieces, SMD_CALL);
#undef SMD_CALL
  } else if (CO == 16) {
#define SMD_CALL(P, T) launch_conv16<P, T>(x, wp_fwd, y, B, C, false, h + 2, w + 2, h, w, st)
    SMD_BY_PIECES(pieces, SMD_CALL);
#undef SMD_CALL
  } else {
#define SMD_CALL(P, T) launch_conv_form<P, 0, T>(x, wp_fwd, y, split_ws, B, C, CO, h + 2, w + 2, h, w, two_tiles, st)
    SMD_BY_PIECES(pieces, SMD_CALL);
#undef SMD_CALL
  }
  return hipGetLastError();
}
hipError_t launch_conv_mfma_bwd_data(const void* gy, const void* wp_bwd, void* g_x, float* split_ws, bool zpad, int B, int C, int CO, int h, int w, int pieces, bool two_tiles, hipStream_t st) {
  if (zpad) {
#define SMD_CALL(P) launch_conv_form<P, 1, float>(gy, wp_bwd, g_x, split_ws, B, CO, C, h, w, h, w, two_tiles, st)
    SMD_BY_PIECES_F32(pieces, SMD_CALL);
#undef SMD_CALL
  } else if (CO == 16 && C == 16) {
#define SMD_CALL(P, T) launch_conv16<P, T>(gy, wp_bwd, g_x, B, 16, true, h, w, h + 2, w + 2, st)
    SMD_BY_PIECES(pieces, SMD_CALL);
#undef SMD_CALL
  } else {
#define SMD_CALL(P, T) launch_conv_form<P, 2, T>(gy, wp_bwd, g_x, split_ws, B, CO, C, h, w, h + 2, w + 2, two_tiles, st)
    SMD_BY_PIECES(pieces, SMD_CALL);
#undef SMD_CALL
  }
  return hipGetLastError();
}
template <int P, typename T>
static void launch_wgrad(const void* xp_, const void* gy_, float* partial, int B, int C, int CO, int h, int w, hipStream_t st) {
  const T* xp = (const T*)xp_; const T* gy = (const T*)gy_;
  dim3 grid; int rows;
  if (CO == 16) {
    wgrad16_shape(B, C, h, w, grid, rows);
    if constexpr (std::is_same<T, float>::value) {
      if (C == 16) hipLaunchKernelGGL((k_conv16_wgrad_dma<1, P>), grid, dim3(128), 0, st, xp, gy, partial, h, w, rows);
      else hipLaunchKernelGGL((k_conv16_wgrad_dma<2, P>), grid, dim3(256), 0, st, xp, gy, partial, h, w, rows);
    } else {
      if (C == 16) hipLaunchKernelGGL((k_conv16_wgrad_mfma<1, P, T>), grid, dim3(128), 0, st, xp, gy, partial, h, w, rows);
      else hipLaunchKernelGGL((k_conv16_wgrad_mfma<2, P, T>), grid, dim3(256), 0, st, xp, gy, partial, h, w, rows);
    }
    return;
  }
  int spb;
  wgrad_shape(B, C, CO, h, w, grid, rows, spb, std::is_same<T, float>::value);
  if constexpr (std::is_same<T, float>::value) hipLaunchKernelGGL((k_conv_wgrad_dma<P, false>), grid, dim3(256), 0, st, xp, gy, partial, B, C, CO, h, w, rows, spb);
  else hipLaunchKernelGGL((k_conv_wgrad_mfma<P, T>), grid, dim3(256), 0, st, xp, gy, partial, C, CO, h, w, rows);
}
static hipError_t wgrad_finalize(float* g_w, float* partial, int B, int C, int CO, int h, int w, bool multi, hipStream_t st) {
  const unsigned T = wgrad_sets(B, C, CO, h, w, multi), G = wgrad_slices(T);
  const int n = CO*C*9;
  double* slice = reinterpret_cast<double*>(partial + (size_t)T*n);
  if (G == 1) hipLaunchKernelGGL(k_conv_wgrad_finalize<true>, dim3(ceil_div(n, 64), 1), dim3(256), 0, st, partial, T, 1u, CO, C, slice, g_w);
  else {
    hipLaunchKernelGGL(k_conv_wgrad_finalize<false>, dim3(ceil_div(n, 64), G), dim3(256), 0, st, partial, T, G, CO, C, slice, g_w);
    hipLaunchKernelGGL(k_conv_wgrad_finalize2, dim3(ceil_div(n, 256)), dim3(256), 0, st, slice, G, CO, C, g_w);
  }
  return hipGetLastError();
}
hipError_t launch_conv_mfma_bwd_wgt(const void* xp, const void* gy, float* g_w, float* partial, bool zpad, int B, int C, int CO, int h, int w, int pieces, hipStream_t st) {
  if (zpad) {
    dim3 grid; int rows, spb;
    wgrad_shape(B, C, CO, h, w, grid, rows, spb, true);
#define SMD_CALL(P) hipLaunchKernelGGL((k_conv_wgrad_dma<P, true>), grid, dim3(256), 0, st, (const float*)xp, (const float*)gy, partial, B, C, CO, h, w, rows, spb)
    SMD_BY_PIECES_F32(pieces, SMD_CALL);
#undef SMD_CALL
  } else {
#define SMD_CALL(P, T) launch_wgrad<P, T>(xp, gy, partial, B, C, CO, h, w, st)
    SMD_BY_PIECES(pieces, SMD_CALL);
#undef SMD_CALL
  }
  return wgrad_finalize(g_w, partial, B, C, CO, h, w, zpad || pieces != 1, st);
}

}

#ifdef SMD_CONV_TRACE
extern "C" int smd_debug_conv_trace(unsigned long long* host_out, int blocks) {
  return (int)hipMemcpyFromSymbol(host_out, HIP_SYMBOL(smd::g_conv_trace), (size_t)blocks*40*sizeof(unsigned long long), 0, hipMemcpyDeviceToHost);
}
#endif
```

### slowtv_monodepth_amd/csrc/smd_kernels.h

```cpp
#pragma once
#include <hip/hip_runtime.h>
#include <stddef.h>
#include <stdint.h>

#include "../../include/smd_hotpath.h"

namespace smd {

constexpr int kFwdCols = 62;
constexpr int kBwdCols = 60;
#ifndef SMD_WAVES_PER_BLOCK
#define SMD_WAVES_PER_BLOCK 4
#endif
constexpr int kWavesPerBlock = SMD_WAVES_PER_BLOCK;
#ifndef SMD_SMOOTH_CHUNK
#define SMD_SMOOTH_CHUNK 1024
#endif
constexpr int kSmoothChunk = SMD_SMOOTH_CHUNK;
__host__ __device__ inline int smooth_chunk_px(int n) { return n > 32768 ? kSmoothChunk : 256; }
__host__ __device__ inline int smooth_chunks_of(int n) { return (n + smooth_chunk_px(n) - 1)/smooth_chunk_px(n); }
constexpr int kSmoothCols = 63, kSmoothRows = 8;
__host__ __device__ inline int smooth_units_of(int hs, int ws) { return ((ws + kSmoothCols - 1)/kSmoothCols)*((hs + kSmoothRows - 1)/kSmoothRows); }
constexpr int kSmoothRowsMain = 16;
__host__ __device__ inline int smooth_units_main(int hs, int ws) { return ((ws + kSmoothCols - 1)/kSmoothCols)*((hs + kSmoothRowsMain - 1)/kSmoothRowsMain); }
constexpr int kPoseSums = 12;

struct ScaleSet {
  const float* p[SMD_MAX_SCALES];
  float* g[SMD_MAX_SCALES];
  int hs[SMD_MAX_SCALES];
  int ws[SMD_MAX_SCALES];
  int key[SMD_MAX_SCALES];
  int S;
};

__host__ __device__ inline size_t packed_texel_floats(int b, int n, int h, int w) { return (size_t)n*b*(size_t)(h + 1)*(size_t)(w + 1)*3; }
__host__ __device__ inline size_t packed_ypix_floats(int b, int h, int w) { return (size_t)b*(size_t)h*(size_t)w*3; }
__host__ __device__ inline size_t packed_tpix_floats(int b, int h, int w) { return (size_t)b*(size_t)h*(size_t)w*4; }
__host__ __device__ inline size_t packed_image_floats(int b, int n, int h, int w) {
  return packed_texel_floats(b, n, h, w) + packed_ypix_floats(b, h, w) + 2*packed_tpix_floats(b, h, w);
}
__host__ __device__ inline size_t packed_rowtab_offset_floats(int b, int n, int h, int w) { return (packed_image_floats(b, n, h, w) + 3) & ~(size_t)3; }
__host__ __device__ inline size_t packed_arrive_offset_floats(int b, int n, int h, int w) { return packed_rowtab_offset_floats(b, n, h, w) + (size_t)SMD_MAX_SCALES*(size_t)(h + 4)*4; }
constexpr int kLiveSupports = 4;
__host__ __device__ inline size_t live_max_strips(int h, int w) { return (size_t)((w + kFwdCols - 1)/kFwdCols)*(size_t)((h + 3)/4); }
__host__ __device__ inline size_t packed_live_offset_floats(int b, int n, int h, int w) { return (packed_arrive_offset_floats(b, n, h, w) + (((size_t)b + 1 + 3) & ~(size_t)3) + 63) & ~(size_t)63; }
__host__ __device__ inline size_t live_header_floats(int b) { return ((size_t)b + 63) & ~(size_t)63; }
__host__ __device__ inline size_t live_table_floats(int b, int h, int w) { return live_header_floats(b) + (size_t)SMD_MAX_SCALES*b*live_max_strips(h, w)*kLiveSupports*2; }
__host__ __device__ inline size_t packed_total_floats(int b, int n, int h, int w) { return packed_live_offset_floats(b, n, h, w) + live_table_floats(b, h, w); }

struct LossCombine { float* out3; unsigned* arrive; float w_rec, w_sm; };
struct SmoothFwdJob {
  const float* edge_w;
  float* partial; int max_units; float* stats; float* loss;
  unsigned* arrive;
  double* contrib;
  LossCombine comb;
};

struct ReconPrepArgs {
  const float* tgt;
  const float* supp;
  float* packed;
  int b, n, h, w;
  int i0, ni;
  int flags;
  int rh, nsx, nsy;
  int first_pass, last_pass;
  uint4* rowtab;
  unsigned* arrive;
  int sc_S, sc_hs[SMD_MAX_SCALES], sc_ws[SMD_MAX_SCALES];
};

struct ReconMainArgs {
  const float* depth;
  float* depth_out;
  ScaleSet sc;
  float a_scale, a_off;
  const uint4* rowtab;
  const float* packed;
  const float* T;
  const float* K;
  const float* Kinv;
  const float* noise;
  float* err;
  uint8_t* sel;
  float* partial;
  unsigned* arrive;
  float* loss;
  double loss_scale;
  float* warp0;
  int b, n, S, h, w;
  int i0, ni;
  int flags;
  int rh;
  int nsx, nsy;
  int b1, rh2, nsy2;
  float wscale, hscale;
  float inv_n;
  uint32_t seed_lo, seed_hi;
  int first_pass, last_pass;
  int lookahead;
  int share;
  int main_blocks, guest_blocks;
  SmoothFwdJob sm;
  LossCombine comb;
  unsigned* live;
};

struct ReconBwdArgs {
  const float* depth; const float* packed; const float* T; const float* K; const float* Kinv;
  const uint8_t* sel;
  const float* g_loss;
  float g_scale;
  float* g_depth;
  const float* g_in;
  float k0_scale;
  float* pose_partial;
  unsigned* arrive;
  float* g_T; float* g_K; float* g_Kinv;
  int b, n, S, h, w;
  int flags;
  int rh, nsx, nsy;
  int b1, rh2, nsy2;
  int pose_stride;
  int wps;
  int scales_block;
  float wscale, hscale;
  int skip_level;
  int pair;
  const unsigned* live;
  int fwd_rh, fwd_b1, fwd_rh2;
  float* g_direct;
  int direct_scale;
};

__host__ __device__ inline int ceil_div(int a, int b) { return (a + b - 1)/b; }

constexpr int SMD_MAX_AR_SEGMENTS = 8;
struct CropResizeArgs {
  const float* src[SMD_MAX_AR_SEGMENTS]; float* dst[SMD_MAX_AR_SEGMENTS];
  int planes[SMD_MAX_AR_SEGMENTS], first_plane[SMD_MAX_AR_SEGMENTS];
  int nseg;
  int H, W;
  int y0, x0, ch, cw;
  int resample;
  int oh, ow;
  const float* K_in; float* K_out; int nK;
};
hipError_t launch_crop_resize(const CropResizeArgs& a, hipStream_t st);

__device__ __forceinline__ void decode_tile(unsigned p, int nbx, int b, int S, int& xb, int& bi, int& s) {
  const unsigned nq = (unsigned)nbx*(unsigned)b, full = nq & ~7u;
  unsigned q;
  if (p < full*(unsigned)S) { const unsigned slot = p >> 3; q = (slot/(unsigned)S)*8u + (p & 7u); s = (int)(slot % (unsigned)S); }
  else { const unsigned r = p - full*(unsigned)S; q = full + r/(unsigned)S; s = (int)(r % (unsigned)S); }
  bi = (int)(q/(unsigned)nbx); xb = (int)(q - (unsigned)bi*(unsigned)nbx);
}

__host__ __device__ inline unsigned recon_grid_blocks(int nstrips, int b, int S, int spb = kWavesPerBlock) {
  return (unsigned)ceil_div(nstrips, spb)*(unsigned)b*(unsigned)S;
}
__device__ __forceinline__ void decode_wave(unsigned p, int wid, int nstrips, int b, int S, int& strip, int& bi, int& s) {
  int xb;
  decode_tile(p, ceil_div(nstrips, kWavesPerBlock), b, S, xb, bi, s);
  strip = xb*kWavesPerBlock + wid;
}

void note_variant(int which, const char* fmt, ...);
hipError_t launch_recon_prep(const ReconPrepArgs& a, hipStream_t st);
hipError_t launch_recon_main(const ReconMainArgs& a, hipStream_t st);
hipError_t launch_recon_bwd(const ReconBwdArgs& a, hipStream_t st);
hipError_t launch_sum_partials(const float* partial, int count, double scale, float* out, hipStream_t st);
hipError_t launch_pose_finalize(const float* pose_partial, int entries, int stride, const float* T, const float* K, const float* Kinv,
                                float* g_T, float* g_K, float* g_Kinv, int b, int n, hipStream_t st);

hipError_t launch_disp_to_depth_fwd(const ScaleSet& sc, int b, int h, int w, float min_depth, float max_depth,
                                    float* depth_up, float* disp_up, hipStream_t st);
struct BwdMap;
size_t disp_to_depth_bwd_tmp_floats(const ScaleSet& sc, int b, int h, int w, BwdMap* map);
struct PoseChain {
  const float* aa; const float* t; const uint8_t* invert; float* g_aa; float* g_t;
  const float* fs; const float* cs; float* g_fs; float* g_cs;
  int h, w;
};
struct SmoothBwdJob { const float* stats; const float* edge_w; const float* g_loss; float g_scale; int blocks_per_sample; int accumulate_scale; };
struct PoseFinJob { ReconBwdArgs a; int entries1, entries2, b1; PoseChain chain; SmoothBwdJob sm; };
hipError_t launch_disp_to_depth_bwd(const ScaleSet& sc, int b, int h, int w, float min_depth, float max_depth,
                                    const float* depth_up, const float* g_depth_up, float* tmp, bool premultiplied, hipStream_t st,
                                    const PoseFinJob* job = nullptr, int skip_scale = -1, bool accumulate = false);

hipError_t launch_smooth_fwd(const ScaleSet& sc, int b, const float* img, int h, int w, int flags, float* loss, float* stats,
                             float* disp_grad, float* image_grad, float* ws_sums, float* edge_w, bool edges_ready, hipStream_t st);
hipError_t launch_blur3(const float* x, float* out, int planes, int h, int w, bool adjoint, hipStream_t st);
hipError_t launch_smooth_edges(const ScaleSet& sc, int b, const float* img, int h, int w, float* edge_w, hipStream_t st);
size_t smooth_edge_bytes(const ScaleSet& sc, int b);
hipError_t launch_smooth_bwd(const ScaleSet& sc, int b, const float* img, int h, int w, int flags, const float* stats,
                             const float* g_loss, const float* edge_w, hipStream_t st, float g_scale = 1.f, int accumulate_scale = -1);
hipError_t launch_smooth_main(const ScaleSet& sc, int b, const SmoothFwdJob& job, hipStream_t st);
void smooth_fwd_job(const ScaleSet& sc, int b, float* loss, float* stats, float* ws_sums, float* edge_w, SmoothFwdJob* job);

hipError_t launch_view_synth_fwd(const float* input, const float* depth, const float* T, const float* K, const float* Kinv,
                                 float* warp, float* depth_warp, uint8_t* mask_valid, int B, int C, int h, int w, hipStream_t st);
hipError_t launch_view_synth_bwd(const float* input, const float* depth, const float* T, const float* K, const float* Kinv,
                                 const float* g_warp, const float* g_depth_warp, float* g_input, float* g_depth,
                                 float* g_T, float* g_K, float* g_Kinv, float* ws, int B, int C, int h, int w, hipStream_t st);
hipError_t launch_photo_error_fwd(const float* pred, const float* target, float* err, int N, int C, int h, int w, int flags, float w_ssim, hipStream_t st);
hipError_t launch_photo_error_bwd(const float* pred, const float* target, const float* g_err, float* g_pred, float* ws,
                                  int N, int C, int h, int w, int flags, float w_ssim, hipStream_t st);
hipError_t launch_recon_reduce_fwd(const float* err_warp, const float* err_static, const float* mask, const float* noise, uint64_t seed,
                                   float* err, uint8_t* sel, float* loss, float* ws, int n, int B, int h, int w, int flags,
                                   hipStream_t st);
hipError_t launch_recon_reduce_bwd(const uint8_t* sel, const float* g_loss, float* g_err_warp, const float* err_warp, const float* err_static,
                                   const float* mask, float* g_mask, int n, int B, int h, int w, int flags, hipStream_t st);
hipError_t launch_debug_lane_shift(float* out_left, float* out_right, hipStream_t st);
hipError_t launch_stream_copy(const void* src, void* dst, size_t nbytes, int mode, hipStream_t st);
size_t conv_head_partials(int B, int C, int h, int w);
hipError_t launch_conv_head_fwd(const void* xp, int x_bf16, const float* wgt, const float* bias, float* y, int B, int C, int h, int w, int act, hipStream_t st);
hipError_t launch_conv_head_bwd(const void* xp, int x_bf16, const float* wgt, const float* y, const float* gy, void* g_xp, float* g_w, float* g_bias, float* partial,
                                int B, int C, int h, int w, int act, hipStream_t st);
size_t conv_headn_partials(int B, int C, int N, int h, int w);
hipError_t launch_conv_headn_fwd(const void* xp, int x_bf16, const float* wgt, const float* bias, float* y, int B, int C, int N, int h, int w, int act, hipStream_t st);
hipError_t launch_conv_headn_bwd(const void* xp, int x_bf16, const float* wgt, const float* y, const float* gy, void* g_xp, float* g_w, float* g_bias, float* partial,
                                 int B, int C, int N, int h, int w, int act, hipStream_t st);
hipError_t launch_upsample_stack_fwd(const ScaleSet& sc, int planes, int h, int w, float* out, hipStream_t st);
hipError_t launch_upsample_stack_bwd(const ScaleSet& sc, int planes, int h, int w, const float* g_out, hipStream_t st);
struct MeanSet {
  const float* p[SMD_MAX_SCALES];
  float* g[SMD_MAX_SCALES];
  long long n[SMD_MAX_SCALES];
  int first_block[SMD_MAX_SCALES + 1];
  int S;
};
int scale_mean_blocks(MeanSet& ms);
hipError_t launch_scale_mean_fwd(MeanSet ms, int mode, float* partial, unsigned* counter, float* loss, hipStream_t st);
hipError_t launch_scale_mean_bwd(MeanSet ms, int mode, const float* g_loss, hipStream_t st);
hipError_t launch_conv_thin_fwd(const float* xp, const float* wgt, float* y, int B, int C, int h, int w, hipStream_t st);
size_t conv_thin_partials(int B, int C, int h, int w);
hipError_t launch_conv_thin_bwd_wgt(const float* xp, const float* gy, float* g_w, float* partial, int B, int C, int h, int w, hipStream_t st);
hipError_t launch_conv_thin_bwd_data(const float* gy, const float* wgt, float* g_xp, int B, int C, int h, int w, hipStream_t st);
enum class ConvOp { Fwd, Data, Wgt };
inline bool conv_mfma_served(ConvOp op, bool zpad, int C, int CO) {
  const bool thin = !zpad && CO == 16 && (C == 16 || C == 32);
  if (op == ConvOp::Fwd) return (C % 16 == 0 && CO % 32 == 0) || thin;
  if (op == ConvOp::Data) return (CO % 16 == 0 && C % 32 == 0) || (thin && C == 16);
  return CO % 32 == 0 || thin;
}
size_t conv_mfma_packed_elems(int C, int CO, int pieces);
size_t conv_mfma_wgrad_partials(bool zpad, int B, int C, int CO, int h, int w);
size_t conv_mfma_split_elems(ConvOp op, bool zpad, int B, int C, int CO, int h, int w, bool two_tiles);
hipError_t launch_conv_mfma_pack(const float* w, void* wp_fwd, void* wp_bwd, int C, int CO, int pieces, hipStream_t st);
hipError_t launch_conv_mfma_fwd(const void* x, const void* wp_fwd, void* y, float* split_ws, bool zpad, int B, int C, int CO, int h, int w, int pieces, bool two_tiles, hipStream_t st);
hipError_t launch_conv_mfma_bwd_data(const void* gy, const void* wp_bwd, void* g_x, float* split_ws, bool zpad, int B, int C, int CO, int h, int w, int pieces, bool two_tiles, hipStream_t st);
hipError_t launch_conv_mfma_bwd_wgt(const void* x, const void* gy, float* g_w, float* partial, bool zpad, int B, int C, int CO, int h, int w, int pieces, hipStream_t st);
bool conv_stem_served(int C, int CO);
size_t conv_stem_packed_bytes(int C);
size_t conv_stem_wgrad_floats(int B, int C, int H, int W);
hipError_t launch_conv_stem_pack(const float* w, void* wp, int C, hipStream_t st);
hipError_t launch_conv_stem_fwd(const float* x, const void* wp, float* y, int B, int C, int H, int W, hipStream_t st);
hipError_t launch_conv_stem_bwd_wgt(const float* x, const float* gy, float* g_w, float* partial, int B, int C, int H, int W, hipStream_t st);
size_t decoder_bias_partials(int B, int C, int h, int w);
hipError_t launch_elu_pad_fwd(const void* x, const float* bias, void* out, int B, int C, int h, int w, int apply_elu, int dt, hipStream_t st);
hipError_t launch_elu_pad_bwd(const void* x, const float* bias, const void* g_out, void* g_x, float* g_bias, float* ws, int B, int C, int h, int w,
                              int apply_elu, int dt, hipStream_t st);
hipError_t launch_elu_up_cat_pad_fwd(const void* a, const float* bias, const void* skip, void* out, int B, int Ca, int Cs, int h, int w, int dt,
                                     hipStream_t st);
hipError_t launch_elu_up_cat_pad_bwd(const void* a, const float* bias, const void* g_out, void* g_a, void* g_skip, float* g_bias, float* ws,
                                     int B, int Ca, int Cs, int h, int w, int dt, hipStream_t st);
int bn_chunks(int N, int HW);
hipError_t launch_bn_fwd(const float* x, const float* residual, const float* gamma, const float* beta, float* running_mean, float* running_var,
                         float momentum, float eps, int relu, float* y, float* save_mean, float* save_invstd, float* ws, int N, int C, int HW,
                         hipStream_t st);
hipError_t launch_bn_bwd(const float* x, const float* y, const float* g_y, const float* gamma, const float* save_mean, const float* save_invstd,
                         int relu, float* g_x, float* g_res, float* g_gamma, float* g_beta, float* ws, int N, int C, int HW, hipStream_t st);
hipError_t launch_maxpool_fwd(const float* x, float* y, uint8_t* idx, size_t planes, int H, int W, hipStream_t st);
hipError_t launch_maxpool_bwd(const float* g_y, const uint8_t* idx, float* g_x, size_t planes, int H, int W, hipStream_t st);
int dwconv_tiles(int H, int W);
hipError_t launch_dwconv7(const float* x, const float* w, const float* bias, float* y, int N, int C, int H, int W, int flip, hipStream_t st);
hipError_t launch_dwconv7_wrw(const float* x, const float* gy, float* gw, float* gb, float* ws, int N, int C, int H, int W, hipStream_t st);
int ln_cf_chunks(size_t npix);
hipError_t launch_ln_cf_fwd(const float* x, const float* gamma, const float* beta, void* y, int y_bf16, float* mean, float* rstd, int N, int C, int HW,
                            float eps, hipStream_t st);
hipError_t launch_ln_cf_bwd(const float* x, const void* g_y, int g_bf16, const float* gamma, const float* mean, const float* rstd, float* g_x, float* g_gamma,
                            float* g_beta, float* ws, int N, int C, int HW, hipStream_t st);
int regr_blocks(size_t N);
hipError_t launch_regression_fwd(const float* pred, const float* target, const uint8_t* mask, size_t N, int flags, float* loss, float* err,
                                 float* stats, float* ws, hipStream_t st);
hipError_t launch_regression_bwd(const float* pred, const float* target, const uint8_t* mask, size_t N, int flags, float* stats,
                                 const float* g_loss, float* g_pred, float* g_target, float* ws, hipStream_t st);
hipError_t launch_pose_fwd(const float* aa, const float* t, const uint8_t* invert, int N, float* T, hipStream_t st);
hipError_t launch_pose_bwd(const float* aa, const float* t, const uint8_t* invert, int N, const float* g_T, float* g_aa, float* g_t, hipStream_t st);
hipError_t launch_intrinsics_fwd(const float* fs, const float* cs, const float* Kin, int b, int h, int w, float* K, float* Kinv, hipStream_t st);
hipError_t launch_intrinsics_bwd(const float* fs, const float* cs, int b, int h, int w, const float* g_K, const float* g_Kinv,
                                 float* g_fs, float* g_cs, hipStream_t st);



inline int pick_rows_per_strip(int b, int S, int h, int w, int cols, int halo) {
  const int nsx = ceil_div(w, cols);
  const long target_waves = 6144;
  const int rh_max = 16;
  (void)cols;
  int best = 8;
  for (int rh = rh_max; rh >= 8; rh -= 4) {
    long waves = (long)nsx*ceil_div(h, rh)*b*S;
    best = rh;
    if (waves >= target_waves) break;
  }
  (void)halo;
  return best;
}

}
```

### slowtv_monodepth_amd/functional.py

```python
from ._device import _stream, call
from .class_ops import _ScaleMean, crop_resize, lane_shift_selftest, photo_error, recon_reduce, regression_loss, scale_mean, upsample_stack, view_synth
from .conv_ops import conv3x3_mfma, conv3x3_same, conv3x3_thin, conv3x3_wide, conv7x7s2_stem
from .conv_routing import _conv_route, conv_routes, set_conv_route
from .geom_ops import intrinsics, inv_intrinsics, pose_matrices
from .net_ops import batch_norm_act, conv3x3_head, conv3x3_headn, dwconv7x7, elu_pad, elu_up_cat_pad, layer_norm_cf, max_pool3x3s2
from .recon_ops import (PreparedFrames, disp_smooth_blurred, disp_smooth_fused, disp_to_depth, gaussian_blur3x3, image_recon_fused, image_recon_fused_disp,
                        image_recon_prep, loss_path_fused, recon_flags, supports_per_pass)
from .row_skip import _RowSkipTuner, dead_tile_shares, dead_wave_shares, row_skip_tuner

__all__ = ['conv3x3_headn', 'upsample_stack', 'scale_mean', 'conv3x3_mfma', 'conv3x3_wide', 'conv3x3_same', 'set_conv_route', 'conv_routes', 'loss_path_fused', 'crop_resize', 'disp_to_depth', 'image_recon_prep', 'PreparedFrames', 'image_recon_fused', 'image_recon_fused_disp', 'disp_smooth_fused', 'view_synth', 'photo_error', 'recon_reduce',
           'lane_shift_selftest', 'recon_flags', 'regression_loss', 'elu_pad', 'elu_up_cat_pad', 'batch_norm_act', 'max_pool3x3s2', 'dwconv7x7', 'layer_norm_cf', 'pose_matrices', 'intrinsics', 'inv_intrinsics',
           'conv3x3_head', 'conv3x3_thin', 'conv7x7s2_stem', 'gaussian_blur3x3', 'disp_smooth_blurred', 'supports_per_pass', 'row_skip_tuner', 'dead_tile_shares', 'dead_wave_shares']
```

### slowtv_monodepth_amd/networks/encoders.py

```python
from __future__ import annotations

import torch
import torch.nn as nn
import torch.nn.functional as F

__all__ = ['create_encoder', 'FeatureInfo', 'ResNetFeatures', 'ConvNeXtFeatures', 'ENCODERS']


class FeatureInfo:
    def __init__(self, channels, reduction): self._c, self._r = list(channels), list(reduction)
    def channels(self): return list(self._c)
    def reduction(self): return list(self._r)


class BatchNormAct2d(nn.BatchNorm2d):
    fused_enabled = True

    def forward(self, x, residual=None, relu: bool = False):
        fused = (self.fused_enabled and x.is_cuda and self.training and x.dtype == torch.float32 and not torch.is_autocast_enabled() and self.affine
                 and self.track_running_stats and self.momentum is not None and x.is_contiguous())
        if not fused:
            y = super().forward(x)
            if residual is not None: y = y + residual
            return F.relu(y, inplace=True) if relu else y
        from .. import functional as HF
        self._pending_batches = getattr(self, '_pending_batches', 0) + 1
        return HF.batch_norm_act(x, self.weight, self.bias, self.running_mean, self.running_var, residual=residual,
                                 momentum=self.momentum, eps=self.eps, relu=relu)

    def flush_counter(self):
        n = getattr(self, '_pending_batches', 0)
        if n and self.num_batches_tracked is not None: self.num_batches_tracked += n
        self._pending_batches = 0

    def _save_to_state_dict(self, destination, prefix, keep_vars):
        self.flush_counter()
        super()._save_to_state_dict(destination, prefix, keep_vars)

    def train(self, mode: bool = True):
        if not mode: self.flush_counter()
        return super().train(mode)


def _conv3x3(conv: nn.Conv2d, x):
    if (conv.stride == (1, 1) and BatchNormAct2d.fused_enabled and x.is_cuda and x.dtype == torch.float32 and conv.weight.dtype == torch.float32
            and not torch.is_autocast_enabled() and x.is_contiguous()):
        from .. import functional as HF
        return HF.conv3x3_same(x, conv.weight)
    return conv(x)


def _stem(conv: nn.Conv2d, x):
    if (BatchNormAct2d.fused_enabled and x.is_cuda and x.dtype == torch.float32 and conv.weight.dtype == torch.float32
            and not torch.is_autocast_enabled() and x.is_contiguous()):
        from .. import functional as HF
        return HF.conv7x7s2_stem(x, conv.weight)
    return conv(x)


class BasicBlock(nn.Module):
    def __init__(self, cin, cout, stride):
        super().__init__()
        self.conv1 = nn.Conv2d(cin, cout, 3, stride, 1, bias=False); self.bn1 = BatchNormAct2d(cout)
        self.conv2 = nn.Conv2d(cout, cout, 3, 1, 1, bias=False); self.bn2 = BatchNormAct2d(cout)
        self.down = None
        if stride != 1 or cin != cout:
            self.down = nn.Sequential(nn.Conv2d(cin, cout, 1, stride, bias=False), BatchNormAct2d(cout))

    def forward(self, x):
        idt = x if self.down is None else self.down(x)
        x = self.bn1(_conv3x3(self.conv1, x), relu=True)
        return self.bn2(_conv3x3(self.conv2, x), residual=idt, relu=True)


class Bottleneck(nn.Module):
    def __init__(self, cin, mid, stride):
        super().__init__()
        cout = mid*4
        self.conv1 = nn.Conv2d(cin, mid, 1, bias=False); self.bn1 = BatchNormAct2d(mid)
        self.conv2 = nn.Conv2d(mid, mid, 3, stride, 1, bias=False); self.bn2 = BatchNormAct2d(mid)
        self.conv3 = nn.Conv2d(mid, cout, 1, bias=False); self.bn3 = BatchNormAct2d(cout)
        self.down = None
        if stride != 1 or cin != cout:
            self.down = nn.Sequential(nn.Conv2d(cin, cout, 1, stride, bias=False), BatchNormAct2d(cout))

    def forward(self, x):
        idt = x if self.down is None else self.down(x)
        x = self.bn1(self.conv1(x), relu=True)
        x = self.bn2(_conv3x3(self.conv2, x), relu=True)
        return self.bn3(self.conv3(x), residual=idt, relu=True)


class ResNetFeatures(nn.Module):
    def __init__(self, layers=(2, 2, 2, 2), bottleneck=False, in_chans=3):
        super().__init__()
        self.conv1 = nn.Conv2d(in_chans, 64, 7, 2, 3, bias=False); self.bn1 = BatchNormAct2d(64)
        self.maxpool = nn.MaxPool2d(3, 2, 1)
        widths, exp = (64, 128, 256, 512), (4 if bottleneck else 1)
        stages, cin = [], 64
        for i, (wd, nb) in enumerate(zip(widths, layers)):
            blocks = []
            for j in range(nb):
                stride = 2 if (j == 0 and i > 0) else 1
                blocks.append(Bottleneck(cin, wd, stride) if bottleneck else BasicBlock(cin, wd, stride))
                cin = wd*exp
            stages.append(nn.Sequential(*blocks))
        self.layers = nn.ModuleList(stages)
        self.feature_info = FeatureInfo([64] + [wd*exp for wd in widths], [2, 4, 8, 16, 32])
        for m in self.modules():
            if isinstance(m, nn.Conv2d): nn.init.kaiming_normal_(m.weight, mode='fan_out', nonlinearity='relu')

    def forward(self, x):
        x = self.bn1(_stem(self.conv1, x), relu=True)
        feats = [x]
        if BatchNormAct2d.fused_enabled and x.is_cuda and x.dtype == torch.float32 and not torch.is_autocast_enabled() and x.is_contiguous():
            from .. import functional as HF
            x = HF.max_pool3x3s2(x)
        else:
            x = self.maxpool(x)
        for layer in self.layers:
            x = layer(x); feats.append(x)
        return feats


def _use_nchw_kernels(x) -> bool:
    return BatchNormAct2d.fused_enabled and x.is_cuda and x.dtype in (torch.float32, torch.bfloat16, torch.float16)


class LayerNorm2d(nn.LayerNorm):
    def forward(self, x):
        if _use_nchw_kernels(x):
            from .. import functional as HF
            with torch.autocast('cuda', enabled=False):
                return HF.layer_norm_cf(x.float().contiguous(), self.weight.float(), self.bias.float(), self.eps)
        return F.layer_norm(x.permute(0, 2, 3, 1), self.normalized_shape, self.weight, self.bias, self.eps).permute(0, 3, 1, 2)


class ConvNeXtBlock(nn.Module):
    def __init__(self, dim, ls_init=1e-6):
        super().__init__()
        self.dw = nn.Conv2d(dim, dim, 7, padding=3, groups=dim)
        self.norm = nn.LayerNorm(dim, eps=1e-6)
        self.fc1 = nn.Linear(dim, 4*dim); self.fc2 = nn.Linear(4*dim, dim)
        self.gamma = nn.Parameter(ls_init*torch.ones(dim))

    def forward(self, x):
        if _use_nchw_kernels(x): return self._forward_nchw(x)
        y = self.dw(x).permute(0, 2, 3, 1)
        y = self.fc2(F.gelu(self.fc1(self.norm(y))))*self.gamma
        return x + y.permute(0, 3, 1, 2)

    def _forward_nchw(self, x):
        from .. import functional as HF
        to_bf16 = torch.is_autocast_enabled() and torch.get_autocast_gpu_dtype() == torch.bfloat16
        with torch.autocast('cuda', enabled=False):
            y = HF.dwconv7x7(x.float().contiguous(), self.dw.weight.float(), self.dw.bias.float())
            y = HF.layer_norm_cf(y, self.norm.weight.float(), self.norm.bias.float(), self.norm.eps,
                                 out_dtype=torch.bfloat16 if to_bf16 else torch.float32)
        y = F.conv2d(y, self.fc1.weight[:, :, None, None], self.fc1.bias)
        y = F.conv2d(F.gelu(y), self.fc2.weight[:, :, None, None], self.fc2.bias)
        return torch.addcmul(x, y, self.gamma.view(1, -1, 1, 1).to(y.dtype))


class ConvNeXtFeatures(nn.Module):
    def __init__(self, depths=(3, 3, 9, 3), dims=(96, 192, 384, 768), in_chans=3):
        super().__init__()
        self.stem = nn.Sequential(nn.Conv2d(in_chans, dims[0], 4, 4), LayerNorm2d(dims[0], eps=1e-6))
        stages = []
        for i, (d, c) in enumerate(zip(depths, dims)):
            mods = []
            if i > 0: mods += [LayerNorm2d(dims[i - 1], eps=1e-6), nn.Conv2d(dims[i - 1], c, 2, 2)]
            mods += [ConvNeXtBlock(c) for _ in range(d)]
            stages.append(nn.Sequential(*mods))
        self.stages = nn.ModuleList(stages)
        self.feature_info = FeatureInfo(dims, [4, 8, 16, 32])
        for m in self.modules():
            if isinstance(m, (nn.Conv2d, nn.Linear)):
                nn.init.trunc_normal_(m.weight, std=0.02)
                if m.bias is not None: nn.init.zeros_(m.bias)

    def forward(self, x):
        x = self.stem(x)
        feats = []
        for st in self.stages:
            x = st(x); feats.append(x)
        return feats


ENCODERS = {
    'resnet18': lambda c: ResNetFeatures((2, 2, 2, 2), False, c),
    'resnet34': lambda c: ResNetFeatures((3, 4, 6, 3), False, c),
    'resnet50': lambda c: ResNetFeatures((3, 4, 6, 3), True, c),
    'convnext_tiny': lambda c: ConvNeXtFeatures((3, 3, 9, 3), (96, 192, 384, 768), c),
    'convnext_small': lambda c: ConvNeXtFeatures((3, 3, 27, 3), (96, 192, 384, 768), c),
    'convnext_base': lambda c: ConvNeXtFeatures((3, 3, 27, 3), (128, 256, 512, 1024), c),
}


def create_encoder(name: str, in_chans: int = 3, pretrained: bool = False) -> nn.Module:
    if name not in ENCODERS: raise KeyError(f'Unknown encoder "{name}". Available: {sorted(ENCODERS)}')
    if pretrained:
        import warnings
        warnings.warn(f'create_encoder({name!r}, pretrained=True): no pretrained weights are available offline, the encoder is randomly initialised; '
                      'load a timm / reference state_dict with slowtv_monodepth_amd.networks.checkpoint.load_reference_state_dict', UserWarning, stacklevel=2)
    return ENCODERS[name](in_chans)
```

Baseline: 934.3.

## Add MFMA stride-2 3x3 conv kernels for ResNet downsampling blocks

Adds a new HIP kernel family for 3x3 stride-2 convolutions covering forward, data-gradient and weight-gradient. It uses phase-decomposed LDS tiling with split-precision MFMA and packed weights, and reuses the existing weight-gradient finalize path. The encoder now sends stride-2 BasicBlock conv1 layers to it instead of the rocm/MIOpen conv2d path. A serve/autotune fallback and static routing rules limit it to channel counts that are multiples of 32 and narrow output rows. In exchange, the weights are packed on every forward call and it adds new kernel code that could be numerically riskier.

```diff
diff --git a/include/smd_hotpath.h b/include/smd_hotpath.h
--- a/include/smd_hotpath.h
+++ b/include/smd_hotpath.h
@@ -192,6 +192,14 @@
 int smd_conv7x7s2_bwd_weight(const float* x, const float* g_y, float* g_weight, void* workspace, size_t workspace_bytes,
                              int B, int C, int CO, int H, int W, void* stream);
 
+size_t smd_conv3x3s2_packed_bytes(int C, int CO);
+size_t smd_conv3x3s2_workspace_bytes(int B, int C, int CO, int H, int W);
+int smd_conv3x3s2_pack(const float* weight, void* wp_fwd, void* wp_bwd, int C, int CO, void* stream);
+int smd_conv3x3s2_fwd(const float* x, const void* wp_fwd, float* y, int B, int C, int CO, int H, int W, void* stream);
+int smd_conv3x3s2_bwd_data(const float* g_y, const void* wp_bwd, float* g_x, int B, int C, int CO, int H, int W, void* stream);
+int smd_conv3x3s2_bwd_weight(const float* x, const float* g_y, float* g_weight, void* workspace, size_t workspace_bytes,
+                             int B, int C, int CO, int H, int W, void* stream);
+
 size_t smd_bn_workspace_bytes(int N, int C, int HW);
 int smd_bn_fwd(const float* x, const float* residual, const float* gamma, const float* beta, float* running_mean, float* running_var,
                float momentum, float eps, int relu, float* y, float* save_mean, float* save_invstd,
diff --git a/slowtv_monodepth_amd/_lib.py b/slowtv_monodepth_amd/_lib.py
--- a/slowtv_monodepth_amd/_lib.py
+++ b/slowtv_monodepth_amd/_lib.py
@@ -87,6 +87,12 @@
     'smd_conv7x7s2_pack': (_i, [_vp]*2 + [_i]*2 + [_vp]),
     'smd_conv7x7s2_fwd': (_i, [_vp]*3 + [_i]*5 + [_vp]),
     'smd_conv7x7s2_bwd_weight': (_i, [_vp]*4 + [_sz] + [_i]*5 + [_vp]),
+    'smd_conv3x3s2_packed_bytes': (_sz, [_i]*2),
+    'smd_conv3x3s2_workspace_bytes': (_sz, [_i]*5),
+    'smd_conv3x3s2_pack': (_i, [_vp]*3 + [_i]*2 + [_vp]),
+    'smd_conv3x3s2_fwd': (_i, [_vp]*3 + [_i]*5 + [_vp]),
+    'smd_conv3x3s2_bwd_data': (_i, [_vp]*3 + [_i]*5 + [_vp]),
+    'smd_conv3x3s2_bwd_weight': (_i, [_vp]*4 + [_sz] + [_i]*5 + [_vp]),
     'smd_conv3x3_head_workspace_bytes': (_sz, [_i]*4),
     'smd_conv3x3_head_fwd': (_i, [_vp]*4 + [_i]*5 + [_vp]),
     'smd_conv3x3_head_bwd': (_i, [_vp]*8 + [_sz] + [_i]*5 + [_vp]),
diff --git a/slowtv_monodepth_amd/conv_ops.py b/slowtv_monodepth_amd/conv_ops.py
--- a/slowtv_monodepth_amd/conv_ops.py
+++ b/slowtv_monodepth_amd/conv_ops.py
@@ -206,3 +206,69 @@
 
 def conv7x7s2_stem(x, weight):
     return _Conv7x7s2Stem.apply(x, weight)
+
+
+def _s2_pack(weight, C, CO, want_fwd, want_bwd):
+    nbytes = _lib.lib.smd_conv3x3s2_packed_bytes(C, CO)
+    wf = _workspace(weight.device, nbytes, floor=256)[0] if want_fwd else None
+    wb = _workspace(weight.device, nbytes, floor=256)[0] if want_bwd else None
+    call('smd_conv3x3s2_pack', weight.data_ptr(), _ptr(wf), _ptr(wb), C, CO, _stream())
+    return wf, wb
+
+
+class _Conv3x3s2(torch.autograd.Function):
+    @staticmethod
+    def forward(ctx, x, weight, force):
+        x = _check('x', x)
+        if x.ndim != 4: raise ValueError(f'expected (B,C,H,W), got {tuple(x.shape)}')
+        B, C, H, W = x.shape
+        if weight.ndim != 4 or tuple(weight.shape[1:]) != (C, 3, 3): raise ValueError(f'weight: expected (CO,{C},3,3), got {tuple(weight.shape)}')
+        CO = weight.shape[0]
+        weight = _check('weight', weight, (CO, C, 3, 3))
+        dims = (B, C, CO, H, W)
+        served = _lib.lib.smd_conv3x3s2_workspace_bytes(*dims) > 0
+        if force and not served: raise _lib.Unsupported(f'the stride-2 kernels serve C % 32 == 0 with CO % 32 == 0 and output rows of at most 128 pixels, not {dims}')
+        y = torch.empty((B, CO, (H - 1)//2 + 1, (W - 1)//2 + 1), device=x.device, dtype=torch.float32)
+        packed = {}
+
+        def run_mfma():
+            packed['wf'], packed['wb'] = _s2_pack(weight, C, CO, True, True)
+            call('smd_conv3x3s2_fwd', x.data_ptr(), packed['wf'].data_ptr(), y.data_ptr(), *dims, _stream())
+            return y
+        out = serve(('fwd_z2', *dims), run_mfma, lambda: torch.conv2d(x, weight, None, 2, 1), eligible=served, force=force)
+        ctx.save_for_backward(x, weight, packed.get('wb'))
+        ctx.served, ctx.force = served, force
+        return out
+
+    @staticmethod
+    def backward(ctx, g_y):
+        x, weight, wp_bwd = ctx.saved_tensors
+        dev = _on(x)
+        B, C, H, W = x.shape
+        CO = weight.shape[0]
+        dims = (B, C, CO, H, W)
+        need_x, need_w = ctx.needs_input_grad[0], ctx.needs_input_grad[1]
+        g_y = _check('grad(y)', g_y, (B, CO, (H - 1)//2 + 1, (W - 1)//2 + 1))
+        cb = lambda mask: torch.ops.aten.convolution_backward(g_y, x, weight, None, [2, 2], [1, 1], [1, 1], False, [0, 0], 1, mask)
+        g_x = g_w = None
+        if need_x:
+            g_x = torch.empty_like(x)
+
+            def run_data():
+                wb = wp_bwd if wp_bwd is not None else _s2_pack(weight, C, CO, False, True)[1]
+                call('smd_conv3x3s2_bwd_data', g_y.data_ptr(), wb.data_ptr(), g_x.data_ptr(), *dims, _stream())
+                return g_x
+            g_x = serve(('data_z2', *dims), run_data, lambda: cb([True, False, False])[0], eligible=ctx.served, force=ctx.force)
+        if need_w:
+            g_w = torch.empty_like(weight)
+
+            def run_wgt():
+                ws, nws = _workspace(dev, _lib.lib.smd_conv3x3s2_workspace_bytes, *dims, floor=256)
+                call('smd_conv3x3s2_bwd_weight', x.data_ptr(), g_y.data_ptr(), g_w.data_ptr(), ws.data_ptr(), nws, *dims, _stream())
+                return g_w
+            g_w = serve(('wgt_z2', *dims), run_wgt, lambda: cb([False, True, False])[1], eligible=ctx.served, force=ctx.force)
+        return g_x, g_w, None
+
+
+def conv3x3_s2(x, weight, force: bool = False):
+    return _Conv3x3s2.apply(x, weight, bool(force))
diff --git a/slowtv_monodepth_amd/conv_routing.py b/slowtv_monodepth_amd/conv_routing.py
--- a/slowtv_monodepth_amd/conv_routing.py
+++ b/slowtv_monodepth_amd/conv_routing.py
@@ -41,9 +41,13 @@
            'coarse': lambda v, B, C, CO, h, w: (w <= _COARSE_W_MAX and C >= _COARSE_C_MIN) == v}
 
 
+STRIDED_SUFFIX = 'z2'
+STRIDED_RULES = {'fwd': [dict(c_max=128)], 'data': [dict(c_max=128)], 'wgt': []}
+
+
 def static_rule(op, B, C, CO, h, w) -> bool:
     kind, _, suffix = op.partition('_')
-    clauses = STATIC_RULES[_FAMILY_OF_SUFFIX[suffix]][kind]
+    clauses = STRIDED_RULES[kind] if suffix == STRIDED_SUFFIX else STATIC_RULES[_FAMILY_OF_SUFFIX[suffix]][kind]
     return any(all(_BOUNDS[name](v, B, C, CO, h, w) for name, v in clause.items()) for clause in clauses)
 
 
diff --git a/slowtv_monodepth_amd/csrc/smd_api.hip b/slowtv_monodepth_amd/csrc/smd_api.hip
--- a/slowtv_monodepth_amd/csrc/smd_api.hip
+++ b/slowtv_monodepth_amd/csrc/smd_api.hip
@@ -946,6 +946,45 @@
   if (workspace_bytes < smd_conv7x7s2_workspace_bytes(B, C, CO, H, W)) return fail(SMD_E_WORKSPACE, "workspace too small");
   return check_launch(smd::launch_conv_stem_bwd_wgt(x, g_y, g_weight, (float*)workspace, B, C, H, W, (hipStream_t)stream), "conv7x7s2_bwd_weight");
 }
+static bool s2_sizes_ok(int B, int C, int CO, int H, int W) {
+  if (B < 1 || B > 65535 || C < 1 || CO < 1 || C > 4096 || CO > 4096 || H < 1 || W < 1 || H >= 32768 || W >= 32768) return false;
+  const long long ho = (H - 1)/2 + 1, wo = (W - 1)/2 + 1;
+  return (long long)B*C*H*W < (1ll << 31) && (long long)B*CO*ho*wo < (1ll << 31) && (long long)B*ho*(CO/32 + C/32) < (1ll << 28);
+}
+static int s2_check(int B, int C, int CO, int H, int W) {
+  if (!s2_sizes_ok(B, C, CO, H, W)) return fail(SMD_E_INVALID, "invalid sizes B=%d C=%d CO=%d H=%d W=%d", B, C, CO, H, W);
+  if (!smd::conv_s2_served(C, CO)) return fail(SMD_E_UNSUPPORTED, "the stride-2 kernels serve C %% 32 == 0 with CO %% 32 == 0, not C=%d CO=%d", C, CO);
+  if (!smd::conv_s2_taken(B, C, CO, H, W)) return fail(SMD_E_UNSUPPORTED, "the stride-2 kernels serve output rows of at most 128 pixels, not W=%d", W);
+  return SMD_OK;
+}
+size_t smd_conv3x3s2_packed_bytes(int C, int CO) { return (C <= 4096 && CO <= 4096 && smd::conv_s2_served(C, CO)) ? align256(smd::conv_s2_packed_bytes(C, CO)) : 0; }
+size_t smd_conv3x3s2_workspace_bytes(int B, int C, int CO, int H, int W) {
+  if (!s2_sizes_ok(B, C, CO, H, W) || !smd::conv_s2_taken(B, C, CO, H, W)) return 0;
+  return align256(std::max((size_t)64, smd::conv_s2_wgrad_floats(B, C, CO, H, W))*sizeof(float));
+}
+int smd_conv3x3s2_pack(const float* weight, void* wp_fwd, void* wp_bwd, int C, int CO, void* stream) {
+  if (!weight || (!wp_fwd && !wp_bwd)) return fail(SMD_E_INVALID, "null pointer");
+  if (C < 1 || CO < 1 || C > 4096 || CO > 4096) return fail(SMD_E_INVALID, "invalid sizes C=%d CO=%d", C, CO);
+  if (!smd::conv_s2_served(C, CO)) return fail(SMD_E_UNSUPPORTED, "the stride-2 kernels serve C %% 32 == 0 with CO %% 32 == 0, not C=%d CO=%d", C, CO);
+  return check_launch(smd::launch_conv_s2_pack(weight, wp_fwd, wp_bwd, C, CO, (hipStream_t)stream), "conv3x3s2_pack");
+}
+int smd_conv3x3s2_fwd(const float* x, const void* wp_fwd, float* y, int B, int C, int CO, int H, int W, void* stream) {
+  if (!x || !wp_fwd || !y) return fail(SMD_E_INVALID, "null pointer");
+  if (int rc = s2_check(B, C, CO, H, W)) return rc;
+  return check_launch(smd::launch_conv_s2_fwd(x, wp_fwd, y, B, C, CO, H, W, (hipStream_t)stream), "conv3x3s2_fwd");
+}
+int smd_conv3x3s2_bwd_data(const float* g_y, const void* wp_bwd, float* g_x, int B, int C, int CO, int H, int W, void* stream) {
+  if (!g_y || !wp_bwd || !g_x) return fail(SMD_E_INVALID, "null pointer");
+  if (int rc = s2_check(B, C, CO, H, W)) return rc;
+  return check_launch(smd::launch_conv_s2_bwd_data(g_y, wp_bwd, g_x, B, C, CO, H, W, (hipStream_t)stream), "conv3x3s2_bwd_data");
+}
+int smd_conv3x3s2_bwd_weight(const float* x, const float* g_y, float* g_weight, void* workspace, size_t workspace_bytes,
+                             int B, int C, int CO, int H, int W, void* stream) {
+  if (!x || !g_y || !g_weight || !workspace) return fail(SMD_E_INVALID, "null pointer");
+  if (int rc = s2_check(B, C, CO, H, W)) return rc;
+  if (workspace_bytes < smd_conv3x3s2_workspace_bytes(B, C, CO, H, W)) return fail(SMD_E_WORKSPACE, "workspace too small");
+  return check_launch(smd::launch_conv_s2_bwd_wgt(x, g_y, g_weight, (float*)workspace, B, C, CO, H, W, (hipStream_t)stream), "conv3x3s2_bwd_weight");
+}
 int smd_elu_up_cat_pad_fwd(const void* a, const float* bias, const void* skip, void* out, int B, int Ca, int Cs, int h, int w, int dtypes, void* stream) {
   if (!a || !out || (Cs > 0 && !skip)) return fail(SMD_E_INVALID, "null pointer");
   if (B < 1 || Ca < 1 || Cs < 0 || h < 1 || w < 1 || !dec_sizes_ok((long long)B*(Ca + Cs), 2*h, 2*w))
diff --git a/slowtv_monodepth_amd/csrc/smd_conv_mfma.hip b/slowtv_monodepth_amd/csrc/smd_conv_mfma.hip
--- a/slowtv_monodepth_amd/csrc/smd_conv_mfma.hip
+++ b/slowtv_monodepth_amd/csrc/smd_conv_mfma.hip
@@ -1138,8 +1138,8 @@
   if constexpr (std::is_same<T, float>::value) hipLaunchKernelGGL((k_conv_wgrad_dma<P, false>), grid, dim3(256), 0, st, xp, gy, partial, B, C, CO, h, w, rows, spb);
   else hipLaunchKernelGGL((k_conv_wgrad_mfma<P, T>), grid, dim3(256), 0, st, xp, gy, partial, C, CO, h, w, rows);
 }
-static hipError_t wgrad_finalize(float* g_w, float* partial, int B, int C, int CO, int h, int w, bool multi, hipStream_t st) {
-  const unsigned T = wgrad_sets(B, C, CO, h, w, multi), G = wgrad_slices(T);
+hipError_t launch_conv_wgrad_finalize(float* g_w, float* partial, unsigned T, int C, int CO, hipStream_t st) {
+  const unsigned G = wgrad_slices(T);
   const int n = CO*C*9;
   double* slice = reinterpret_cast<double*>(partial + (size_t)T*n);
   if (G == 1) hipLaunchKernelGGL(k_conv_wgrad_finalize<true>, dim3(ceil_div(n, 64), 1), dim3(256), 0, st, partial, T, 1u, CO, C, slice, g_w);
@@ -1148,6 +1148,10 @@
     hipLaunchKernelGGL(k_conv_wgrad_finalize2, dim3(ceil_div(n, 256)), dim3(256), 0, st, slice, G, CO, C, g_w);
   }
   return hipGetLastError();
+}
+size_t conv_wgrad_set_floats(unsigned T, int C, int CO) { return wgrad_floats(T, C, CO); }
+static hipError_t wgrad_finalize(float* g_w, float* partial, int B, int C, int CO, int h, int w, bool multi, hipStream_t st) {
+  return launch_conv_wgrad_finalize(g_w, partial, wgrad_sets(B, C, CO, h, w, multi), C, CO, st);
 }
 hipError_t launch_conv_mfma_bwd_wgt(const void* xp, const void* gy, float* g_w, float* partial, bool zpad, int B, int C, int CO, int h, int w, int pieces, hipStream_t st) {
   if (zpad) {
diff --git a/slowtv_monodepth_amd/csrc/smd_conv_s2.hip b/slowtv_monodepth_amd/csrc/smd_conv_s2.hip
--- /dev/null
+++ b/slowtv_monodepth_amd/csrc/smd_conv_s2.hip
@@ -0,0 +1,369 @@
+#include "smd_common.h"
+#include "smd_kernels.h"
+#include "smd_split_dev.h"
+#include <algorithm>
+
+namespace smd {
+
+namespace {
+
+constexpr int kFwdSlots = 1152, kDataSlots = 512;
+constexpr int kStripDw = 20;
+
+__host__ __device__ constexpr int s2_data_tap(int s, int g) {
+  return s == 0 ? (g == 0 ? 4 : -1) : s == 1 ? (g == 0 ? 3 : 5) : s == 2 ? (g == 0 ? 1 : 7) : s == 3 ? (g == 0 ? 0 : 2) : (g == 0 ? 6 : 8);
+}
+__host__ __device__ constexpr int s2_data_phase(int s) { return s < 3 ? s : 3; }
+
+__global__ __launch_bounds__(256) void k_s2_pack_w(const float* __restrict__ w, uint4* __restrict__ wf, uint4* __restrict__ wb, int CO, int C) {
+  const int per = (CO >> 5)*(C >> 3)*320;
+  const int idx = blockIdx.x*256 + threadIdx.x;
+  if (idx >= 2*per) return;
+  const bool data = idx >= per;
+  uint4* dst = data ? wb : wf;
+  if (!dst) return;
+  const int i = data ? idx - per : idx;
+  const int lane = i & 63, s = (i >> 6) % 5, rest = i/320;
+  const int KC = (data ? CO : C) >> 3, kc = rest % KC, mt = rest/KC;
+  const int m = mt*32 + (lane & 31), g = lane >> 5;
+  const int tap = data ? s2_data_tap(s, g) : (2*s + g < 9 ? 2*s + g : -1);
+  float v[8];
+#pragma unroll
+  for (int e = 0; e < 8; ++e) {
+    const int k = kc*8 + e, co = data ? k : m, c = data ? m : k;
+    v[e] = tap >= 0 ? w[((size_t)co*C + c)*9 + tap] : 0.f;
+  }
+  unsigned pk[4][3];
+#pragma unroll
+  for (int q = 0; q < 4; ++q) split_pair<3>(v[2*q], v[2*q + 1], pk[q]);
+#pragma unroll
+  for (int p = 0; p < 3; ++p) dst[((size_t)(i >> 6)*3 + p)*64 + lane] = uint4{pk[0][p], pk[1][p], pk[2][p], pk[3][p]};
+}
+
+template <bool DATA, int NF>
+__global__ __launch_bounds__(256, 2) void k_s2_conv(const float* __restrict__ in, const uint4* __restrict__ wp, float* __restrict__ out, int CK, int M, int B,
+                                                    int H, int W, int ho, int wo, int R, int S, unsigned nbands, unsigned ngroups) {
+  static_assert(!DATA || NF == 1, "the data gradient keeps one fragment per wave");
+  constexpr int SLOTS = DATA ? kDataSlots : kFwdSlots, TRIPS = (SLOTS + 255)/256, NACC = DATA ? 4 : NF, NPROD = n_products(3);
+  __shared__ uint4 tile[3*SLOTS];
+  const int lane = threadIdx.x & 63, wv = __builtin_amdgcn_readfirstlane(threadIdx.x >> 6), j = lane & 31, g = lane >> 5;
+  const int MT = M >> 5;
+  const unsigned nblk = (unsigned)MT*nbands*ngroups, per = (nblk + 7)/8;
+  const unsigned lid = (blockIdx.x & 7)*per + (blockIdx.x >> 3);
+  if (lid >= nblk) return;
+  const int mt = (int)(lid % MT);
+  const unsigned tl = lid/MT;
+  const int y0 = (int)(tl % nbands)*R, b0 = (int)(tl/nbands)*S;
+  const int PW = wo + 1;
+  const int SEG = DATA ? (R + 1)*PW : (2*R + 1)*2*PW;
+  const int hi = DATA ? ho : H, wi = DATA ? wo : W, plane = hi*wi;
+
+  int lbase[NF], pb[NF], py_[NF], px_[NF];
+#pragma unroll
+  for (int nf = 0; nf < NF; ++nf) {
+    const int p = (wv*NF + nf)*32 + j, spx = R*wo;
+    const int seg = p/spx, q = p - seg*spx, ry = q/wo, x = q - ry*wo;
+    const bool ok = seg < S && b0 + seg < B && y0 + ry < ho;
+    pb[nf] = ok ? b0 + seg : -1; py_[nf] = y0 + ry; px_[nf] = x;
+    lbase[nf] = ok ? seg*SEG + (DATA ? ry*PW + x : 4*ry*PW + x) : 0;
+  }
+  int toff[5];
+#pragma unroll
+  for (int s = 0; s < 5; ++s) {
+    const int tap = DATA ? (g ? s2_data_tap(s, 1) : s2_data_tap(s, 0)) : (2*s + g < 9 ? 2*s + g : -1);
+    const int ky = tap/3, kx = tap - 3*ky;
+    toff[s] = tap < 0 ? 0 : DATA ? (ky == 0 ? PW : 0) + (kx == 0 ? 1 : 0) : (2*ky + (kx & 1))*PW + (kx >> 1);
+  }
+
+  const int nitems = S*SEG;
+  int pofs[TRIPS], slot[TRIPS];
+#pragma unroll
+  for (int t = 0; t < TRIPS; ++t) {
+    const int item = t*256 + (int)threadIdx.x;
+    slot[t] = -1; pofs[t] = -1;
+    if (item < nitems) {
+      const int seg = item/SEG, rem = item - seg*SEG;
+      int yy, xx;
+      if (DATA) { const int pr = rem/PW, pc = rem - pr*PW; yy = y0 + pr; xx = pc; slot[t] = item; }
+      else { const int pr = rem/(2*PW), pc = rem - pr*2*PW; yy = 2*y0 - 1 + pr; xx = pc - 1; slot[t] = seg*SEG + (pr*2 + (pc & 1))*PW + (pc >> 1); }
+      if (b0 + seg < B && yy >= 0 && yy < hi && xx >= 0 && xx < wi) pofs[t] = (b0 + seg)*CK*plane + yy*wi + xx;
+    }
+  }
+  float v[TRIPS][8];
+  auto request = [&](int kc) {
+#pragma unroll
+    for (int t = 0; t < TRIPS; ++t) {
+      const float* p = in + (size_t)kc*8*plane + (size_t)max(pofs[t], 0);
+#pragma unroll
+      for (int e = 0; e < 8; ++e) v[t][e] = pofs[t] >= 0 ? p[(size_t)e*plane] : 0.f;
+    }
+  };
+  auto file = [&]() {
+#pragma unroll
+    for (int t = 0; t < TRIPS; ++t) {
+      if (slot[t] >= 0) {
+        unsigned pk[4][3];
+#pragma unroll
+        for (int q = 0; q < 4; ++q) split_pair<3>(v[t][2*q], v[t][2*q + 1], pk[q]);
+#pragma unroll
+        for (int p = 0; p < 3; ++p) tile[p*SLOTS + slot[t]] = uint4{pk[0][p], pk[1][p], pk[2][p], pk[3][p]};
+      }
+    }
+  };
+
+  f32x16 acc[NACC], lo[NACC];
+#pragma unroll
+  for (int a = 0; a < NACC; ++a)
+#pragma unroll
+    for (int r = 0; r < 16; ++r) { acc[a][r] = 0.f; lo[a][r] = 0.f; }
+
+  const int KC = CK >> 3;
+  const uint4* wq = wp + (size_t)mt*KC*15*64 + lane;
+  request(0);
+  for (int kc = 0; kc < KC; ++kc) {
+    bf16x8 A[3][3];
+    auto fetch_a = [&](int s) {
+#pragma unroll
+      for (int p = 0; p < 3; ++p) A[s % 3][p] = as_frag(wq[(size_t)((kc*5 + s)*3 + p)*64]);
+    };
+    fetch_a(0); fetch_a(1); fetch_a(2);
+    file();
+    __syncthreads();
+#pragma unroll
+    for (int s = 0; s < 5; ++s) {
+      bf16x8 Bf[NF][3];
+#pragma unroll
+      for (int nf = 0; nf < NF; ++nf)
+#pragma unroll
+        for (int p = 0; p < 3; ++p) Bf[nf][p] = as_frag(tile[p*SLOTS + lbase[nf] + toff[s]]);
+#pragma unroll
+      for (int t = 0; t < NPROD; ++t)
+#pragma unroll
+        for (int nf = 0; nf < NF; ++nf) {
+          const int a = DATA ? s2_data_phase(s) : nf;
+          if (t == NPROD - 1) acc[a] = __builtin_amdgcn_mfma_f32_32x32x16_bf16(A[s % 3][0], Bf[nf][0], acc[a], 0, 0, 0);
+          else lo[a] = __builtin_amdgcn_mfma_f32_32x32x16_bf16(A[s % 3][prod_a(3, t)], Bf[nf][prod_b(3, t)], lo[a], 0, 0, 0);
+        }
+      if (s < 2) fetch_a(s + 3);
+      if (s == 1 && kc + 1 < KC) request(kc + 1);
+      __builtin_amdgcn_sched_barrier(0);
+    }
+    __syncthreads();
+  }
+
+  if (DATA) {
+    if (pb[0] >= 0) {
+#pragma unroll
+      for (int ph = 0; ph < 4; ++ph) {
+        const int iy = 2*py_[0] + (ph >> 1), ix = 2*px_[0] + (ph & 1);
+        if (iy < H && ix < W) {
+#pragma unroll
+          for (int rr = 0; rr < 16; ++rr) {
+            const int m = mt*32 + (rr & 3) + 8*(rr >> 2) + 4*g;
+            out[(((size_t)pb[0]*M + m)*H + iy)*W + ix] = acc[ph][rr] + lo[ph][rr];
+          }
+        }
+      }
+    }
+  } else {
+#pragma unroll
+    for (int nf = 0; nf < NF; ++nf) {
+      if (pb[nf] >= 0) {
+#pragma unroll
+        for (int rr = 0; rr < 16; ++rr) {
+          const int m = mt*32 + (rr & 3) + 8*(rr >> 2) + 4*g;
+          out[(((size_t)pb[nf]*M + m)*ho + py_[nf])*wo + px_[nf]] = acc[nf][rr] + lo[nf][rr];
+        }
+      }
+    }
+  }
+}
+
+__global__ __launch_bounds__(256, 2) void k_s2_wgrad(const float* __restrict__ x, const float* __restrict__ gy, float* __restrict__ partial, int C, int CO,
+                                                     int H, int W, int ho, int wo, int GR, int RB, int CT) {
+  constexpr int NPROD = n_products(3), DW = kStripDw;
+  __shared__ __attribute__((aligned(16))) unsigned gs[3*64*DW];
+  __shared__ __attribute__((aligned(16))) unsigned xs[3*3*64*DW];
+  const int lane = threadIdx.x & 63, wv = __builtin_amdgcn_readfirstlane(threadIdx.x >> 6), j = lane & 31, g = lane >> 5;
+  const int wm = wv & 1, wn = wv >> 1;
+  const int c0 = (int)(blockIdx.x % CT)*64, co0 = (int)(blockIdx.x/CT)*64;
+  const int g0 = blockIdx.y*RB, nrows = min(RB, GR - g0), nstrips = ceil_div(wo, 32), NU = nrows*nstrips;
+
+  float xv[4][5], gv[2][4];
+  auto load_x = [&](int u, int ky) {
+    const int gr = g0 + u/nstrips, x0 = (u % nstrips)*32, b = gr/ho, iy = 2*(gr - b*ho) + ky - 1;
+#pragma unroll
+    for (int t = 0; t < 4; ++t) {
+      const int item = t*256 + (int)threadIdx.x, cl = item >> 4, tt = item & 15;
+      const int c = min(c0 + cl, C - 1), col = 2*(x0 + 2*tt) - 1;
+      const float* row = x + (((size_t)b*C + c)*H + max(iy, 0))*W;
+      const bool ok = iy >= 0 && iy < H;
+#pragma unroll
+      for (int k = 0; k < 5; ++k) xv[t][k] = (ok && col + k >= 0 && col + k < W) ? row[col + k] : 0.f;
+    }
+  };
+  auto file_x = [&]() {
+#pragma unroll
+    for (int t = 0; t < 4; ++t) {
+      const int item = t*256 + (int)threadIdx.x, cl = item >> 4, tt = item & 15;
+      unsigned p0[3], p1[3], p2[3];
+      split_pair<3>(xv[t][0], xv[t][2], p0);
+      split_pair<3>(xv[t][1], xv[t][3], p1);
+      split_pair<3>(xv[t][2], xv[t][4], p2);
+#pragma unroll
+      for (int p = 0; p < 3; ++p) {
+        xs[((p*3 + 0)*64 + cl)*DW + tt] = p0[p];
+        xs[((p*3 + 1)*64 + cl)*DW + tt] = p1[p];
+        xs[((p*3 + 2)*64 + cl)*DW + tt] = p2[p];
+      }
+    }
+  };
+  auto load_g = [&](int u) {
+    const int gr = g0 + u/nstrips, x0 = (u % nstrips)*32, b = gr/ho, yy = gr - b*ho;
+#pragma unroll
+    for (int t = 0; t < 2; ++t) {
+      const int item = t*256 + (int)threadIdx.x, col = item >> 3, q = item & 7;
+      const int co = min(co0 + col, CO - 1), xa = x0 + 4*q;
+      const float* row = gy + (((size_t)b*CO + co)*ho + yy)*wo;
+#pragma unroll
+      for (int k = 0; k < 4; ++k) gv[t][k] = (xa + k < wo) ? row[xa + k] : 0.f;
+    }
+  };
+  auto file_g = [&]() {
+#pragma unroll
+    for (int t = 0; t < 2; ++t) {
+      const int item = t*256 + (int)threadIdx.x, col = item >> 3, q = item & 7;
+      unsigned p0[3], p1[3];
+      split_pair<3>(gv[t][0], gv[t][1], p0);
+      split_pair<3>(gv[t][2], gv[t][3], p1);
+#pragma unroll
+      for (int p = 0; p < 3; ++p) {
+        gs[(p*64 + col)*DW + 2*q] = p0[p];
+        gs[(p*64 + col)*DW + 2*q + 1] = p1[p];
+      }
+    }
+  };
+
+  f32x16 acc[9];
+#pragma unroll
+  for (int t = 0; t < 9; ++t)
+#pragma unroll
+    for (int r = 0; r < 16; ++r) acc[t][r] = 0.f;
+
+  load_x(0, 0); load_g(0);
+  for (int u = 0; u < NU; ++u) {
+    const int nks = (wo - (u % nstrips)*32) > 16 ? 2 : 1;
+#pragma unroll
+    for (int ky = 0; ky < 3; ++ky) {
+      file_x();
+      if (ky == 0) file_g();
+      __syncthreads();
+      if (ky < 2) load_x(u, ky + 1);
+      else if (u + 1 < NU) { load_x(u + 1, 0); load_g(u + 1); }
+#pragma unroll
+      for (int ks = 0; ks < 2; ++ks) {
+        if (ks < nks) {
+          bf16x8 A[3];
+#pragma unroll
+          for (int p = 0; p < 3; ++p) A[p] = as_frag(*reinterpret_cast<const uint4*>(&gs[(p*64 + wm*32 + j)*DW + ks*8 + g*4]));
+#pragma unroll
+          for (int kx = 0; kx < 3; ++kx) {
+            bf16x8 Bf[3];
+#pragma unroll
+            for (int p = 0; p < 3; ++p) Bf[p] = as_frag(*reinterpret_cast<const uint4*>(&xs[((p*3 + kx)*64 + wn*32 + j)*DW + ks*8 + g*4]));
+#pragma unroll
+            for (int t = 0; t < NPROD; ++t)
+              acc[ky*3 + kx] = __builtin_amdgcn_mfma_f32_32x32x16_bf16(A[prod_a(3, t)], Bf[prod_b(3, t)], acc[ky*3 + kx], 0, 0, 0);
+          }
+        }
+      }
+      __syncthreads();
+    }
+  }
+
+  const int c = c0 + wn*32 + j;
+  if (c < C) {
+#pragma unroll
+    for (int t = 0; t < 9; ++t)
+#pragma unroll
+      for (int r = 0; r < 16; ++r) {
+        const int co = co0 + wm*32 + (r & 3) + 8*(r >> 2) + 4*g;
+        if (co < CO) partial[(((size_t)blockIdx.y*9 + t)*CO + co)*C + c] = acc[t][r];
+      }
+  }
+}
+
+struct S2Band { int R, S; unsigned nbands, ngroups; };
+bool s2_band(bool data, int B, int ho, int wo, int npb, S2Band& sb) {
+  if (wo > npb) return false;
+  const int slots = data ? kDataSlots : kFwdSlots, PW = wo + 1;
+  auto seg = [&](int R) { return data ? (R + 1)*PW : (2*R + 1)*2*PW; };
+  int R = std::min(ho, std::max(1, npb/wo));
+  while (R > 1 && seg(R) > slots) --R;
+  if (seg(R) > slots) return false;
+  int S = 1;
+  if (R == ho) S = std::max(1, std::min({npb/(ho*wo), slots/seg(R), B}));
+  sb = S2Band{R, S, (unsigned)ceil_div(ho, R), (unsigned)ceil_div(B, S)};
+  return true;
+}
+int s2_fwd_nf(int B, int CO, int ho, int wo, S2Band& sb) {
+#ifndef SMD_S2_FORCE_NF1
+  if (s2_band(false, B, ho, wo, 256, sb) && (long long)(CO >> 5)*sb.nbands*sb.ngroups >= 384) return 2;
+#endif
+  return s2_band(false, B, ho, wo, 128, sb) ? 1 : 0;
+}
+void s2_wgrad_shape(int B, int C, int CO, int ho, dim3& grid, int& RB, int& CT) {
+  CT = ceil_div(C, 64);
+  const int tiles = CT*ceil_div(CO, 64), GR = B*ho;
+  const int nb = std::min(GR, std::max(1, 512/tiles));
+  RB = std::max(ceil_div(GR, nb), std::min(2, GR));
+  grid = dim3(tiles, ceil_div(GR, RB));
+}
+
+}
+
+bool conv_s2_served(int C, int CO) { return C >= 32 && CO >= 32 && C % 32 == 0 && CO % 32 == 0; }
+bool conv_s2_taken(int B, int C, int CO, int H, int W) {
+  const int ho = (H - 1)/2 + 1, wo = (W - 1)/2 + 1;
+  S2Band sb;
+  return conv_s2_served(C, CO) && wo <= 128 && s2_fwd_nf(B, CO, ho, wo, sb) > 0 && s2_band(true, B, ho, wo, 128, sb);
+}
+size_t conv_s2_packed_bytes(int C, int CO) { return (size_t)(CO >> 5)*(C >> 3)*5*3*1024; }
+size_t conv_s2_wgrad_floats(int B, int C, int CO, int H, int W) {
+  dim3 grid; int RB, CT;
+  s2_wgrad_shape(B, C, CO, (H - 1)/2 + 1, grid, RB, CT);
+  return conv_wgrad_set_floats(grid.y, C, CO);
+}
+hipError_t launch_conv_s2_pack(const float* w, void* wp_fwd, void* wp_bwd, int C, int CO, hipStream_t st) {
+  const int n = 2*(CO >> 5)*(C >> 3)*320;
+  hipLaunchKernelGGL(k_s2_pack_w, dim3(ceil_div(n, 256)), dim3(256), 0, st, w, (uint4*)wp_fwd, (uint4*)wp_bwd, CO, C);
+  return hipGetLastError();
+}
+hipError_t launch_conv_s2_fwd(const float* x, const void* wp_fwd, float* y, int B, int C, int CO, int H, int W, hipStream_t st) {
+  const int ho = (H - 1)/2 + 1, wo = (W - 1)/2 + 1;
+  S2Band sb;
+  const int nf = s2_fwd_nf(B, CO, ho, wo, sb);
+  if (!nf) return hipErrorInvalidValue;
+  const unsigned nblk = (unsigned)(CO >> 5)*sb.nbands*sb.ngroups;
+  const dim3 grid(8*((nblk + 7)/8));
+  if (nf == 2) hipLaunchKernelGGL((k_s2_conv<false, 2>), grid, dim3(256), 0, st, x, (const uint4*)wp_fwd, y, C, CO, B, H, W, ho, wo, sb.R, sb.S, sb.nbands, sb.ngroups);
+  else hipLaunchKernelGGL((k_s2_conv<false, 1>), grid, dim3(256), 0, st, x, (const uint4*)wp_fwd, y, C, CO, B, H, W, ho, wo, sb.R, sb.S, sb.nbands, sb.ngroups);
+  return hipGetLastError();
+}
+hipError_t launch_conv_s2_bwd_data(const float* gy, const void* wp_bwd, float* g_x, int B, int C, int CO, int H, int W, hipStream_t st) {
+  const int ho = (H - 1)/2 + 1, wo = (W - 1)/2 + 1;
+  S2Band sb;
+  if (!s2_band(true, B, ho, wo, 128, sb)) return hipErrorInvalidValue;
+  const unsigned nblk = (unsigned)(C >> 5)*sb.nbands*sb.ngroups;
+  hipLaunchKernelGGL((k_s2_conv<true, 1>), dim3(8*((nblk + 7)/8)), dim3(256), 0, st, gy, (const uint4*)wp_bwd, g_x, CO, C, B, H, W, ho, wo, sb.R, sb.S, sb.nbands, sb.ngroups);
+  return hipGetLastError();
+}
+hipError_t launch_conv_s2_bwd_wgt(const float* x, const float* gy, float* g_w, float* partial, int B, int C, int CO, int H, int W, hipStream_t st) {
+  const int ho = (H - 1)/2 + 1, wo = (W - 1)/2 + 1;
+  dim3 grid; int RB, CT;
+  s2_wgrad_shape(B, C, CO, ho, grid, RB, CT);
+  hipLaunchKernelGGL(k_s2_wgrad, grid, dim3(256), 0, st, x, gy, partial, C, CO, H, W, ho, wo, B*ho, RB, CT);
+  return launch_conv_wgrad_finalize(g_w, partial, grid.y, C, CO, st);
+}
+
+}
diff --git a/slowtv_monodepth_amd/csrc/smd_kernels.h b/slowtv_monodepth_amd/csrc/smd_kernels.h
--- a/slowtv_monodepth_amd/csrc/smd_kernels.h
+++ b/slowtv_monodepth_amd/csrc/smd_kernels.h
@@ -259,6 +259,16 @@
 hipError_t launch_conv_stem_pack(const float* w, void* wp, int C, hipStream_t st);
 hipError_t launch_conv_stem_fwd(const float* x, const void* wp, float* y, int B, int C, int H, int W, hipStream_t st);
 hipError_t launch_conv_stem_bwd_wgt(const float* x, const float* gy, float* g_w, float* partial, int B, int C, int H, int W, hipStream_t st);
+size_t conv_wgrad_set_floats(unsigned T, int C, int CO);
+hipError_t launch_conv_wgrad_finalize(float* g_w, float* partial, unsigned T, int C, int CO, hipStream_t st);
+bool conv_s2_served(int C, int CO);
+bool conv_s2_taken(int B, int C, int CO, int H, int W);
+size_t conv_s2_packed_bytes(int C, int CO);
+size_t conv_s2_wgrad_floats(int B, int C, int CO, int H, int W);
+hipError_t launch_conv_s2_pack(const float* w, void* wp_fwd, void* wp_bwd, int C, int CO, hipStream_t st);
+hipError_t launch_conv_s2_fwd(const float* x, const void* wp_fwd, float* y, int B, int C, int CO, int H, int W, hipStream_t st);
+hipError_t launch_conv_s2_bwd_data(const float* gy, const void* wp_bwd, float* g_x, int B, int C, int CO, int H, int W, hipStream_t st);
+hipError_t launch_conv_s2_bwd_wgt(const float* x, const float* gy, float* g_w, float* partial, int B, int C, int CO, int H, int W, hipStream_t st);
 size_t decoder_bias_partials(int B, int C, int h, int w);
 hipError_t launch_elu_pad_fwd(const void* x, const float* bias, void* out, int B, int C, int h, int w, int apply_elu, int dt, hipStream_t st);
 hipError_t launch_elu_pad_bwd(const void* x, const float* bias, const void* g_out, void* g_x, float* g_bias, float* ws, int B, int C, int h, int w,
diff --git a/slowtv_monodepth_amd/functional.py b/slowtv_monodepth_amd/functional.py
--- a/slowtv_monodepth_amd/functional.py
+++ b/slowtv_monodepth_amd/functional.py
@@ -1,6 +1,6 @@
 from ._device import _stream, call
 from .class_ops import _ScaleMean, crop_resize, lane_shift_selftest, photo_error, recon_reduce, regression_loss, scale_mean, upsample_stack, view_synth
-from .conv_ops import conv3x3_mfma, conv3x3_same, conv3x3_thin, conv3x3_wide, conv7x7s2_stem
+from .conv_ops import conv3x3_mfma, conv3x3_s2, conv3x3_same, conv3x3_thin, conv3x3_wide, conv7x7s2_stem
 from .conv_routing import _conv_route, conv_routes, set_conv_route
 from .geom_ops import intrinsics, inv_intrinsics, pose_matrices
 from .net_ops import batch_norm_act, conv3x3_head, conv3x3_headn, dwconv7x7, elu_pad, elu_up_cat_pad, layer_norm_cf, max_pool3x3s2
@@ -10,4 +10,4 @@
 
 __all__ = ['conv3x3_headn', 'upsample_stack', 'scale_mean', 'conv3x3_mfma', 'conv3x3_wide', 'conv3x3_same', 'set_conv_route', 'conv_routes', 'loss_path_fused', 'crop_resize', 'disp_to_depth', 'image_recon_prep', 'PreparedFrames', 'image_recon_fused', 'image_recon_fused_disp', 'disp_smooth_fused', 'view_synth', 'photo_error', 'recon_reduce',
            'lane_shift_selftest', 'recon_flags', 'regression_loss', 'elu_pad', 'elu_up_cat_pad', 'batch_norm_act', 'max_pool3x3s2', 'dwconv7x7', 'layer_norm_cf', 'pose_matrices', 'intrinsics', 'inv_intrinsics',
-           'conv3x3_head', 'conv3x3_thin', 'conv7x7s2_stem', 'gaussian_blur3x3', 'disp_smooth_blurred', 'supports_per_pass', 'row_skip_tuner', 'dead_tile_shares', 'dead_wave_shares']
+           'conv3x3_head', 'conv3x3_thin', 'conv7x7s2_stem', 'conv3x3_s2', 'gaussian_blur3x3', 'disp_smooth_blurred', 'supports_per_pass', 'row_skip_tuner', 'dead_tile_shares', 'dead_wave_shares']
diff --git a/slowtv_monodepth_amd/networks/encoders.py b/slowtv_monodepth_amd/networks/encoders.py
--- a/slowtv_monodepth_amd/networks/encoders.py
+++ b/slowtv_monodepth_amd/networks/encoders.py
@@ -43,10 +43,12 @@
 
 
 def _conv3x3(conv: nn.Conv2d, x):
-    if (conv.stride == (1, 1) and BatchNormAct2d.fused_enabled and x.is_cuda and x.dtype == torch.float32 and conv.weight.dtype == torch.float32
+    if (conv.stride in ((1, 1), (2, 2)) and BatchNormAct2d.fused_enabled and x.is_cuda and x.dtype == torch.float32 and conv.weight.dtype == torch.float32
             and not torch.is_autocast_enabled() and x.is_contiguous()):
         from .. import functional as HF
-        return HF.conv3x3_same(x, conv.weight)
+        if conv.stride == (1, 1): return HF.conv3x3_same(x, conv.weight)
+        if (conv.kernel_size == (3, 3) and conv.padding == (1, 1) and conv.groups == 1 and conv.dilation == (1, 1) and conv.bias is None
+                and conv.padding_mode == 'zeros'): return HF.conv3x3_s2(x, conv.weight)
     return conv(x)
 
 
```

Result: no change. 945.7, median of 6 (+1.2%).
